# kuleshov-group/PlantCaduceus

Measured on AMD Instinct MI355X. Metric: 512-bp sequences/sec (zero-shot logits), PlantCaduceus_l32, higher is better.
Workload: dtype bf16; 1 GPU; PlantCaduceus_l32 (d_model=1024, n_layer=32) bf16 zero-shot SNP scoring: masked-LM forward of 1024 synthetic 512-bp windows per GPU per step (both strands), logits at index 255 -> softmax(a,c,g,t); synthetic checkpoint seed 1234; batch_per_gpu=1024, seq_len=512, parallelism=dp1 (batch-sharded, all_gather of [B,4])

## Files before the change

### plantcaduceus_amd/csrc/api.hip

```cpp
#include <cstdarg>
#include <cstdio>
#include <cstdlib>
#include <cstring>
#include <map>
#include <string>

#include "build_hash.h"
#include "pcad_internal.hpp"

using namespace pcad;

static thread_local char g_err[512] = "";

int pcad::fail(int code, const char* fmt, ...) {
    va_list ap;
    va_start(ap, fmt);
    vsnprintf(g_err, sizeof(g_err), fmt, ap);
    va_end(ap);
    return code;
}

int pcad::positions_arg(const char* who, const int32_t* positions, int P, int L, Positions* pos) {
    if (P < 0 || P > PCAD_MAX_POSITIONS || (P > 0 && !positions)) return fail(PCAD_ERR_INVALID, "%s: bad positions (P=%d)", who, P);
    pos->n = P;
    for (int i = 0; i < 16; ++i) pos->p[i] = 0;
    for (int i = 0; i < P; ++i) {
        if (positions[i] < 0 || positions[i] >= L) return fail(PCAD_ERR_INVALID, "%s: position %d out of range [0,%d)", who, positions[i], L);
        pos->p[i] = positions[i];
    }
    return PCAD_OK;
}

int pcad::probs_cols_arg(const char* who, const int32_t* cols, int vocab, ProbCols* out) {
    if (!cols) return fail(PCAD_ERR_INVALID, "%s: null cols", who);
    for (int j = 0; j < 4; ++j) {
        if (cols[j] < 0 || cols[j] >= vocab) return fail(PCAD_ERR_INVALID, "%s: cols[%d]=%d outside [0, %d)", who, j, cols[j], vocab);
        out->c[j] = cols[j];
    }
    return PCAD_OK;
}

struct Carver {
    char* base;
    size_t off = 0;
    explicit Carver(void* b) : base((char*)b) {}
    void* take(size_t bytes) {
        void* p = base ? base + off : nullptr;
        off += align_up(bytes);
        return p;
    }
};

bool pcad::fold_wanted(const pcad_engine* e) {
    const bool want = e->norm_fold == 1 || (e->norm_fold < 0 && e->cfg.dtype == PCAD_BF16);
    return want && !e->untied && e->rdt == F32 && e->xzsplit && e->blocked;
}

bool pcad::split_wanted(const pcad_engine* e) {
    return e->f32_split && e->cfg.dtype == PCAD_F32 && !fold_wanted(e) && e->xzsplit && e->blocked && e->D % 64 == 0 && e->E % 64 == 0;
}

static int64_t chunk_row_limit(const pcad_engine* e) {
    const int64_t per_row = (int64_t)e->E * e->esz;
    return ((((int64_t)1 << 32) - ((int64_t)2 << 20)) / per_row) & ~(int64_t)7;
}

static void carve_weights(pcad_engine* e, Carver& c) {
    const size_t D = e->D, E = e->E, N = e->N, V = e->V, esz = e->esz;
    const bool pf = fold_wanted(e);
    const bool ps = split_wanted(e);
    e->emb = c.take(V * D * esz);
    e->emb_f32 = (float*)c.take(V * D * 4);
    e->normf_w = (float*)c.take(D * 4);
    e->comp = (int32_t*)c.take(8 * 4);
    e->xz_tab0 = pf ? c.take(V * 2 * E * esz) : nullptr;
    e->layers.resize(e->nl);
    for (auto& L : e->layers) {
        L.norm_w = (float*)c.take(D * 4);
        L.convw = (float*)c.take(convx_packed_bytes((int)E, e->cfg.dtype));
        L.W_in = c.take(2 * E * D * esz);
        L.W_in_f = pf ? c.take(2 * E * D * esz) : nullptr;
        L.W_out = c.take(D * E * esz);
        L.W_out_p = pf && (size_t)fold_padded_width((int)D) != D ? c.take((size_t)fold_padded_width((int)D) * E * esz) : L.W_out;
        L.W_in_s = ps ? c.take(2 * E * 2 * D * 2) : nullptr;
        L.W_out_s = ps ? c.take(D * 2 * E * 2) : nullptr;
        L.W_in_r = e->untied ? c.take(2 * E * D * esz) : nullptr;
        L.W_out_r = e->untied ? c.take(D * E * esz) : nullptr;
        L.W_in_s_r = e->untied && ps ? c.take(2 * E * 2 * D * 2) : nullptr;
        L.W_out_s_r = e->untied && ps ? c.take(D * 2 * E * 2) : nullptr;
        for (int d = 0; d < 2; ++d) {
            DirWeights& w = L.dir[d];
            w.conv_w = (float*)c.take(E * 4 * 4);
            w.conv_b = (float*)c.take(E * 4);
            w.Wx = c.take((size_t)e->XP * E * esz);
            w.Wx_s = ps && e->convx ? c.take((size_t)e->XP * 2 * E * 2) : nullptr;
            w.Wdt = c.take(E * (size_t)e->Rp * esz);
            w.Wdt_s = ps && e->convx ? c.take(E * (size_t)e->Rp * 2 * 2) : nullptr;
            w.dt_bias = (float*)c.take(E * 4);
            w.A2 = (float*)c.take(E * N * 4);
            w.Dskip = (float*)c.take(E * 4);
        }
    }
}

SmallForms pcad::small_forms(const pcad_engine* e, int B, int L) {
    SmallForms f;
    if (!e->segments) return f;
    f.G = scan_segments(2 * B, L, e->E, nullptr);
    f.pair = e->convx && scan_pair_wanted(2 * B, L, e->E);
    f.ksplit = e->convx ? convx_ksplit(2 * B, L, e->E, e->cfg.dtype) : 1;
    return f;
}

Workspace pcad::carve_workspace(const pcad_engine* e, void* base, int Bc, int L, int Bpol) {
    Carver c(base);
    const size_t rows = (size_t)2 * Bc * L;
    const size_t D = e->D, E = e->E, esz = e->esz;
    Workspace w;
    const size_t Dp = fold_padded_width((int)D);
    w.res = c.take(rows * Dp * (e->rdt == F32 ? 4 : esz));
    const bool sp = split_wanted(e);
    w.u = c.take(rows * Dp * esz);
    w.h = c.take(rows * D * esz);
    const size_t rows8 = (rows + 7) / 8 * 8;
    w.xz = c.take((e->xzsplit ? rows8 : rows * 2) * E * esz);
    w.zb = e->xzsplit ? c.take(rows8 * E * esz) : nullptr;
    w.xc[0] = c.take(rows8 * E * esz);
    w.xc[1] = c.take(rows8 * E * esz);
    const size_t dtl_bytes = sp && e->convx ? rows * e->Rp * 2 * 2 : rows * e->Rp * esz;
    w.dtl[0] = c.take(dtl_bytes);
    w.dtl[1] = c.take(dtl_bytes);
    w.bc[0] = (float*)c.take(rows * 2 * e->N * 4);
    w.bc[1] = (float*)c.take(rows * 2 * e->N * 4);
    w.y = c.take(rows8 * E * esz);
    w.ys = sp ? c.take(rows8 * 2 * E * 2) : nullptr;
    w.rstd = (float*)c.take(rows * 4);
    w.ssq = (float*)c.take(rows * (Dp / 128) * 4);
    const SmallForms f = small_forms(e, Bpol, L);
    w.seg = f.G > 1 ? (float*)c.take(scan_segment_bytes(2 * Bc, L, (int)E, 2 * Bpol)) : nullptr;
    w.pair = f.pair ? (float*)c.take(scan_pair_bytes(2 * Bc, (int)E)) : nullptr;
    w.cxp = f.ksplit > 1 ? (float*)c.take(convx_split_bytes(2 * Bc, L, (int)E, e->cfg.dtype, e->Rp, 2 * Bpol)) : nullptr;
    w.xz2 = e->untied ? c.take((e->xzsplit ? rows8 : rows * 2) * E * esz) : nullptr;
    w.zb2 = e->untied && e->xzsplit ? c.take(rows8 * E * esz) : nullptr;
    w.bytes = c.off;
    return w;
}

static const char* const kClassNames[PCAD_NUM_KERNEL_CLASSES] = {
    "add_rmsnorm", "gemm_in_proj", "conv1d_bidir", "gemm_x_proj", "selective_scan", "gemm_out_proj", "final_head",
    "gemm_out_proj_res", "rstd_reduce"};

hipEvent_t pcad::prof_event(pcad_engine* e) {
    if (!e->prof_pool.empty()) {
        hipEvent_t ev = e->prof_pool.back();
        e->prof_pool.pop_back();
        return ev;
    }
    hipEvent_t ev = nullptr;
    if (hipEventCreate(&ev) != hipSuccess) return nullptr;
    return ev;
}

static const pcad_tensor* find(const std::map<std::string, const pcad_tensor*>& m, const std::string& k) {
    auto it = m.find(k);
    return it == m.end() ? nullptr : it->second;
}

static int64_t numel(const pcad_tensor* t) {
    int64_t n = 1;
    for (int i = 0; i < t->ndim; ++i) n *= t->shape[i];
    return n;
}

int pcad::chunk_for(const pcad_engine* e, int B, int L) {
    int64_t cap = chunk_row_limit(e) / (2 * (int64_t)L);
    if (e->chunk > 0 && e->chunk < cap) cap = e->chunk;
    if (cap < 1) cap = 1;
    if (cap > B) cap = B;
    if (e->ws_limit > 0 && carve_workspace(e, nullptr, (int)cap, L, B).bytes > (size_t)e->ws_limit) {
        int64_t lo = 1, hi = cap;
        while (lo < hi) {
            const int64_t mid = (lo + hi + 1) / 2;
            if (carve_workspace(e, nullptr, (int)mid, L, B).bytes <= (size_t)e->ws_limit) lo = mid; else hi = mid - 1;
        }
        cap = lo;
    }
    int64_t n = (B + cap - 1) / cap;
    if (e->chunk == 0 && e->ws_limit == 0) {
        auto whole = [&](int64_t m) { const int64_t c = (B + m - 1) / m; return (2 * c * (int64_t)L) % 16384 == 0; };
        if (!whole(n))
            for (int64_t m = n + 1; m <= 2 * n && m <= B; ++m)
                if (whole(m)) { n = m; break; }
    }
    return (int)((B + n - 1) / n);
}

extern "C" {

int pcad_version(void) { return PCAD_VERSION; }
const char* pcad_build_hash(void) { return PCAD_BUILD_HASH; }
const char* pcad_last_error(void) { return g_err; }

int pcad_create(const pcad_config* cfg, pcad_handle* out) {
    if (!cfg || !out) return fail(PCAD_ERR_INVALID, "pcad_create: null argument");
    if (cfg->d_state != 16) return fail(PCAD_ERR_INVALID, "d_state=%d unsupported (16 only)", cfg->d_state);
    if (cfg->d_conv != 4) return fail(PCAD_ERR_INVALID, "d_conv=%d unsupported (4 only)", cfg->d_conv);
    if (cfg->vocab != 8) return fail(PCAD_ERR_INVALID, "padded vocab=%d unsupported (8 only)", cfg->vocab);
    if (cfg->d_model <= 0 || cfg->d_model % 64 || cfg->d_model > 2048)
        return fail(PCAD_ERR_INVALID, "d_model=%d must be a multiple of 64, <= 2048", cfg->d_model);
    if (cfg->expand < 1) return fail(PCAD_ERR_INVALID, "expand=%d must be >= 1", cfg->expand);
    if (cfg->n_layer < 1) return fail(PCAD_ERR_INVALID, "n_layer=%d must be >= 1", cfg->n_layer);
    if (cfg->dt_rank < 1 || cfg->dt_rank > 256) return fail(PCAD_ERR_INVALID, "dt_rank=%d must be in 1 .. 256", cfg->dt_rank);
    if (cfg->dtype != PCAD_F32 && cfg->dtype != PCAD_BF16) return fail(PCAD_ERR_INVALID, "bad dtype %d", cfg->dtype);
    for (int i = 0; i < 8; ++i)
        if (cfg->complement[i] < 0 || cfg->complement[i] > 7) return fail(PCAD_ERR_INVALID, "bad complement map");
    pcad_engine* e = new pcad_engine();
    e->cfg = *cfg;
    e->D = cfg->d_model; e->E = cfg->expand * cfg->d_model; e->N = 16; e->R = cfg->dt_rank; e->V = 8;
    e->nl = cfg->n_layer;
    e->Rp = padded_dt_rank(e->R);
    e->XP = e->Rp + 2 * e->N;
    e->esz = cfg->dtype == PCAD_BF16 ? 2 : 4;
    e->rdt = (cfg->residual_in_fp32 || cfg->dtype == PCAD_F32) ? F32 : BF16;
    const char* ck = dev_env("PCAD_CHUNK_SEQS");
    e->chunk = ck ? atoi(ck) : 0;
    if (e->chunk < 0) e->chunk = 0;
    e->chunk_rows = 0;
    e->blocked = dev_env("PCAD_PLAIN_LAYOUT") == nullptr && (e->E * e->esz) % 128 == 0;
    e->xzsplit = e->blocked && dev_env("PCAD_PLAIN_XZ") == nullptr && e->E % 16 == 0;
    e->convx = e->xzsplit && (e->Rp == 64 || e->Rp == 96) && dev_env("PCAD_NO_CONVX") == nullptr;
    e->gate_once = true;
    *out = e;
    return PCAD_OK;
}

void pcad_destroy(pcad_handle h) {
    if (!h) return;
    for (int c = 0; c < PCAD_NUM_KERNEL_CLASSES; ++c)
        for (auto& pr : h->prof_ev[c]) { (void)hipEventDestroy(pr.first); (void)hipEventDestroy(pr.second); }
    for (auto ev : h->prof_pool) (void)hipEventDestroy(ev);
    delete h;
}

int pcad_set_option(pcad_handle h, const char* key, int64_t value) {
    if (!h || !key) return fail(PCAD_ERR_INVALID, "pcad_set_option: null argument");
    const std::string k(key);
    if (k == "chunk_seqs") {
        if (value < 0 || value > (1 << 20)) return fail(PCAD_ERR_INVALID, "chunk_seqs=%lld out of range", (long long)value);
        h->chunk = (int)value;
    } else if (k == "gate_each") {
        h->gate_once = value == 0;
    } else if (k == "norm_fold") {
        h->norm_fold = value < 0 ? -1 : (value != 0 ? 1 : 0);
    } else if (k == "workspace_limit_mb") {
        if (value < 0 || value > ((int64_t)1 << 30)) return fail(PCAD_ERR_INVALID, "workspace_limit_mb=%lld out of range", (long long)value);
        h->ws_limit = value << 20;
    } else if (k == "f32_gemm_split") {
        h->f32_split = value != 0;
    } else if (k == "untied_directions") {
        h->untied = value != 0;
    } else if (k == "reference_order") {
        if (value < 0 || value > 2) return fail(PCAD_ERR_INVALID, "reference_order=%lld out of range (0, 1, 2)", (long long)value);
        h->ref_order = (int)value;
        h->gate_once = value == 0;
        h->norm_fold = value == 0 ? -1 : 0;
    } else if (k == "debug_repeat_class") {
        if (value < -1 || value >= PCAD_NUM_KERNEL_CLASSES) return fail(PCAD_ERR_INVALID, "debug_repeat_class=%lld out of range", (long long)value);
        h->rep_class = (int)value;
    } else if (k == "debug_repeat") {
        if (value < 1 || value > 10000) return fail(PCAD_ERR_INVALID, "debug_repeat=%lld out of range", (long long)value);
        h->rep_count = (int)value;
    } else if (k == "poison_workspace") {
        h->poison = value != 0;
    } else if (k == "scan_segments") {
        h->segments = value != 0;
    } else if (k == "last_layer_shortcut") {
        h->shortcut = value != 0;
    } else {
        return fail(PCAD_ERR_INVALID, "pcad_set_option: unknown option '%s'", key);
    }
    return PCAD_OK;
}

int pcad_set_status_buffer(pcad_handle h, int32_t* status) {
    if (!h) return fail(PCAD_ERR_INVALID, "pcad_set_status_buffer: null handle");
    if (((uintptr_t)status) % 4) return fail(PCAD_ERR_INVALID, "pcad_set_status_buffer: misaligned pointer");
    h->status = status;
    return PCAD_OK;
}

size_t pcad_weight_arena_bytes(pcad_handle h) {
    if (!h) return 0;
    pcad_engine tmp = *h;
    Carver c(nullptr);
    carve_weights(&tmp, c);
    return c.off;
}

int pcad_bind_weights(pcad_handle h, const pcad_tensor* tensors, int n, void* arena, size_t arena_bytes,
                      pcad_stream stream) {
    if (!h || !tensors || !arena) return fail(PCAD_ERR_INVALID, "pcad_bind_weights: null argument");
    if (((uintptr_t)arena) % 256) return fail(PCAD_ERR_WORKSPACE, "weight arena must be 256-byte aligned");
    if (arena_bytes < pcad_weight_arena_bytes(h))
        return fail(PCAD_ERR_WORKSPACE, "weight arena too small: %zu < %zu", arena_bytes, pcad_weight_arena_bytes(h));
    hipStream_t s = (hipStream_t)stream;
    pcad_engine* e = h;
    Carver c(arena);
    carve_weights(e, c);
    std::map<std::string, const pcad_tensor*> m;
    for (int i = 0; i < n; ++i) {
        if (!tensors[i].name || !tensors[i].data) return fail(PCAD_ERR_INVALID, "tensor %d has null name/data", i);
        if (tensors[i].dtype != PCAD_F32 && tensors[i].dtype != PCAD_BF16)
            return fail(PCAD_ERR_INVALID, "tensor %s: bad dtype", tensors[i].name);
        m[tensors[i].name] = &tensors[i];
    }
    const int D = e->D, E = e->E, N = e->N, R = e->R, Rp = e->Rp, V = e->V, dt = e->cfg.dtype;
    const std::string pre = "caduceus.backbone.";

    auto need = [&](const std::string& k, int64_t expect, const char* missing_fmt = nullptr) -> const pcad_tensor* {
        const pcad_tensor* t = find(m, k);
        if (!t) {
            if (missing_fmt) fail(PCAD_ERR_INVALID, missing_fmt, k.c_str()); else fail(PCAD_ERR_MISSING, "missing tensor %s", k.c_str());
            return nullptr;
        }
        if (numel(t) != expect) {
            fail(PCAD_ERR_INVALID, "tensor %s has %lld elements, expected %lld", k.c_str(), (long long)numel(t),
                 (long long)expect);
            return nullptr;
        }
        return t;
    };
#define NEED(var, key, ...)                              \
    const pcad_tensor* var = need((key), __VA_ARGS__);   \
    if (!var) return g_err[0] == 'm' ? PCAD_ERR_MISSING : PCAD_ERR_INVALID

    NEED(t_emb, pre + "embeddings.word_embeddings.embedding.weight", (int64_t)V * D);
    HIP_TRY(launch_pack2d(t_emb->data, t_emb->dtype, D, e->emb, dt, D, V, D, V, D, s));
    HIP_TRY(launch_pack2d(e->emb, dt, D, e->emb_f32, F32, D, V, D, V, D, s));
    NEED(t_nf, pre + "norm_f.weight", (int64_t)D);
    HIP_TRY(launch_pack2d(t_nf->data, t_nf->dtype, D, e->normf_w, F32, D, 1, D, 1, D, s));
    HIP_TRY(hipMemcpyAsync(e->comp, e->cfg.complement, 8 * sizeof(int32_t), hipMemcpyHostToDevice, s));

    for (int i = 0; i < e->nl; ++i) {
        LayerWeights& L = e->layers[i];
        const std::string lp = pre + "layers." + std::to_string(i) + ".";
        NEED(t_norm, lp + "norm.weight", (int64_t)D);
        HIP_TRY(launch_pack2d(t_norm->data, t_norm->dtype, D, L.norm_w, F32, D, 1, D, 1, D, s));
        const std::string mf = lp + "mixer.submodule.mamba_fwd.";
        NEED(t_in, mf + "in_proj.weight", (int64_t)2 * E * D);
        HIP_TRY(launch_pack2d(t_in->data, t_in->dtype, D, L.W_in, dt, D, 2 * E, D, 2 * E, D, s));
        if (L.W_in_f) HIP_TRY(launch_pack_scale_cols(t_in->data, t_in->dtype, D, L.norm_w, L.W_in_f, dt, D, 2 * E, D, s));
        NEED(t_out, mf + "out_proj.weight", (int64_t)D * E);
        HIP_TRY(launch_pack2d(t_out->data, t_out->dtype, E, L.W_out, dt, E, D, E, D, E, s));
        if (L.W_out_p != L.W_out) HIP_TRY(launch_pack2d(t_out->data, t_out->dtype, E, L.W_out_p, dt, E, D, E, fold_padded_width(D), E, s));
        if (L.W_in_s) HIP_TRY(launch_pack_split_w(t_in->data, t_in->dtype, D, L.W_in_s, 2 * E, D, s));
        if (L.W_out_s) HIP_TRY(launch_pack_split_w(t_out->data, t_out->dtype, E, L.W_out_s, D, E, s));
        if (e->untied) {
            const std::string mr = lp + "mixer.submodule.mamba_rev.";
            NEED(t_in_r, mr + "in_proj.weight", (int64_t)2 * E * D, "\"untied_directions\" 1 needs tensor %s");
            NEED(t_out_r, mr + "out_proj.weight", (int64_t)D * E, "\"untied_directions\" 1 needs tensor %s");
            HIP_TRY(launch_pack2d(t_in_r->data, t_in_r->dtype, D, L.W_in_r, dt, D, 2 * E, D, 2 * E, D, s));
            HIP_TRY(launch_pack2d(t_out_r->data, t_out_r->dtype, E, L.W_out_r, dt, E, D, E, D, E, s));
            if (L.W_in_s_r) HIP_TRY(launch_pack_split_w(t_in_r->data, t_in_r->dtype, D, L.W_in_s_r, 2 * E, D, s));
            if (L.W_out_s_r) HIP_TRY(launch_pack_split_w(t_out_r->data, t_out_r->dtype, E, L.W_out_s_r, D, E, s));
        }
        for (int d = 0; d < 2; ++d) {
            DirWeights& w = L.dir[d];
            const std::string mp = lp + "mixer.submodule.mamba_" + (d == 0 ? "fwd." : "rev.");
            NEED(t_cw, mp + "conv1d.weight", (int64_t)E * 4);
            HIP_TRY(launch_pack2d(t_cw->data, t_cw->dtype, 4, w.conv_w, F32, 4, E, 4, E, 4, s));
            NEED(t_cb, mp + "conv1d.bias", (int64_t)E);
            HIP_TRY(launch_pack2d(t_cb->data, t_cb->dtype, E, w.conv_b, F32, E, 1, E, 1, E, s));
            NEED(t_x, mp + "x_proj.weight", (int64_t)(R + 2 * N) * E);
            const size_t esz_src = t_x->dtype == PCAD_BF16 ? 2 : 4;
            HIP_TRY(launch_pack2d(t_x->data, t_x->dtype, E, w.Wx, dt, E, R, E, Rp, E, s));
            HIP_TRY(launch_pack2d((const char*)t_x->data + (size_t)R * E * esz_src, t_x->dtype, E,
                                  (char*)w.Wx + (size_t)Rp * E * e->esz, dt, E, 2 * N, E, 2 * N, E, s));
            if (w.Wx_s) HIP_TRY(launch_pack_convx_wsplit((const float*)w.Wx, E, w.Wx_s, e->XP, E, s));
            NEED(t_dw, mp + "dt_proj.weight", (int64_t)E * R);
            HIP_TRY(launch_pack2d(t_dw->data, t_dw->dtype, R, w.Wdt, dt, Rp, E, R, E, Rp, s));
            if (w.Wdt_s) HIP_TRY(launch_pack_split_w(w.Wdt, dt, Rp, w.Wdt_s, E, Rp, s));
            NEED(t_db, mp + "dt_proj.bias", (int64_t)E);
            HIP_TRY(launch_pack2d(t_db->data, t_db->dtype, E, w.dt_bias, F32, E, 1, E, 1, E, s));
            NEED(t_A, mp + "A_log", (int64_t)E * N);
            HIP_TRY(launch_pack_A(t_A->data, t_A->dtype, w.A2, (int64_t)E * N, 1.4426950408889634f, s));
            NEED(t_D, mp + "D", (int64_t)E);
            HIP_TRY(launch_pack2d(t_D->data, t_D->dtype, E, w.Dskip, F32, E, 1, E, 1, E, s));
        }
        if ((E * e->esz) % 128 == 0)
            HIP_TRY(launch_pack_convw(L.dir[0].conv_w, L.dir[0].conv_b, L.dir[1].conv_w, L.dir[1].conv_b, L.convw, E, dt, s));
    }
#undef NEED
    if (e->xz_tab0) HIP_TRY(launch_embed_inproj_table(e->emb, e->layers[0].W_in_f, e->xz_tab0, V, D, 2 * E, e->cfg.eps, dt, s));
    e->fold_packed = fold_wanted(e);
    e->split_packed = split_wanted(e);
    e->untied_packed = e->untied;
    e->bound = true;
    return PCAD_OK;
}

size_t pcad_workspace_bytes(pcad_handle h, int batch, int seqlen) {
    if (!h || batch <= 0 || seqlen <= 0) return 0;
    return carve_workspace(h, nullptr, chunk_for(h, batch, seqlen), seqlen, batch).bytes;
}

int pcad_profile_enable(pcad_handle h, int on) {
    if (!h) return fail(PCAD_ERR_INVALID, "pcad_profile_enable: null handle");
    h->prof = on != 0;
    h->prof_stride = on > 1 ? on : 1;
    for (int c = 0; c < PCAD_NUM_KERNEL_CLASSES; ++c) h->prof_seen[c] = 0;
    return PCAD_OK;
}

int pcad_profile_read(pcad_handle h, pcad_kernel_stat* out, int max_out) {
    if (!h || !out) return fail(PCAD_ERR_INVALID, "pcad_profile_read: null argument");
    for (int c = 0; c < PCAD_NUM_KERNEL_CLASSES; ++c) {
        for (auto& pr : h->prof_ev[c]) {
            HIP_TRY(hipEventSynchronize(pr.second));
            float ms = 0.f;
            HIP_TRY(hipEventElapsedTime(&ms, pr.first, pr.second));
            h->prof_ms[c] += ms;
            h->prof_n[c] += 1;
            h->prof_pool.push_back(pr.first);
            h->prof_pool.push_back(pr.second);
        }
        h->prof_ev[c].clear();
    }
    int n = 0;
    for (int c = 0; c < PCAD_NUM_KERNEL_CLASSES && n < max_out; ++c, ++n) {
        snprintf(out[n].name, sizeof(out[n].name), "%s", kClassNames[c]);
        out[n].launches = h->prof_n[c];
        out[n].total_ms = h->prof_ms[c];
        h->prof_n[c] = 0;
        h->prof_ms[c] = 0.0;
    }
    return n;
}
}
```

### plantcaduceus_amd/csrc/forward.hip

```cpp
#include "pcad_internal.hpp"
using namespace pcad;

namespace {
enum class Head { lm, pooled, loss, probs, layers };
struct ForwardRequest {
    Head head = Head::lm;
    const int32_t* ids = nullptr; int B = 0, L = 0;
    void* workspace = nullptr; size_t ws_bytes = 0; pcad_stream stream = nullptr;
    const int32_t* positions = nullptr; int P = 0;
    const int32_t* pos_per_window = nullptr; int Pw = 0;
    void* all_hidden = nullptr;
    void* hidden_out = nullptr; float* logits_out = nullptr;
    struct {
        int pooling, num_labels;
        const float* score_w; float *pooled_out, *logits_out;
    } pool = {};
    struct {
        const int32_t* labels; const float* loss_weights; int ignore_index;
        float *sums_out, *nll_out, *logits_out;
    } loss = {};
    struct {
        ProbCols cols; float *probs_out, *logits_out;
    } probs = {};
    struct {
        const int32_t* layers;
        int NL;
        bool inter, average;
        int top;
        void* out;
    } lay = {};
};

struct ForwardPlan {
    int chunk, nchunks;
    bool fold, sp, untied;
    bool lay_inter, strict;
    int depth;
    int walk_len;
    SmallForms forms;
    bool tab0;
    int Q;
};

ForwardPlan plan_forward(const pcad_engine* e, const ForwardRequest& rq, const Positions& pos) {
    const int B = rq.B, L = rq.L, D = e->D, E = e->E, P = rq.P;
    ForwardPlan pl;
    pl.Q = rq.pos_per_window ? rq.Pw : (P ? P : L);
    pl.chunk = chunk_for(e, B, L);
    pl.nchunks = (B + pl.chunk - 1) / pl.chunk;
    pl.lay_inter = rq.head == Head::layers && rq.lay.inter;
    pl.fold = fold_wanted(e) && e->fold_packed && !rq.all_hidden && !pl.lay_inter;
    for (int ck = 0; ck < pl.nchunks && pl.fold; ++ck) {
        const int Bc = (B - ck * pl.chunk) < pl.chunk ? (B - ck * pl.chunk) : pl.chunk;
        pl.fold = gemm_fold_shapes_ok((int64_t)2 * Bc * L, D, E, e->cfg.dtype);
    }
    pl.untied = e->untied && e->untied_packed;
    pl.sp = split_wanted(e) && e->split_packed;
    pl.strict = (e->ref_order == 2 || pl.untied) && !pl.fold;
    pl.forms = small_forms(e, B, L);
    pl.depth = pl.lay_inter && rq.lay.top < e->nl ? rq.lay.top : e->nl;
    const bool truncated = pl.depth < e->nl;
    pl.walk_len = 0;
    if (e->shortcut && P > 0 && !rq.pos_per_window && !rq.all_hidden && (int64_t)P * E <= (int64_t)L * D &&
        (truncated ? pl.depth > 0 && !(pl.forms.pair && !pl.strict) : !pl.lay_inter)) {
        int pmin = pos.p[0], pmax = pos.p[0];
        for (int i = 1; i < P; ++i) { pmin = pos.p[i] < pmin ? pos.p[i] : pmin; pmax = pos.p[i] > pmax ? pos.p[i] : pmax; }
        const int need = (pmax + 1 > L - pmin) ? pmax + 1 : L - pmin;
        pl.walk_len = (need + 7) / 8 * 8;
        if (pl.walk_len > L) pl.walk_len = L;
    }
    static const bool tab0 = dev_env("PCAD_NO_TAB0") == nullptr;
    pl.tab0 = tab0;
    return pl;
}

struct Lane { Workspace w; int b0, Bc; };
struct Walk {
    pcad_engine* const e;
    const ForwardRequest& rq; const ForwardPlan& pl; const Positions& pos; const hipStream_t s;
    const int B, L, P, D, E, N, Rp, XP, dt, rdt;
    const int Dp;
    const size_t esz; const float eps;
    const int layP;
    Walk(pcad_engine* e_, const ForwardRequest& rq_, const ForwardPlan& pl_, const Positions& pos_)
        : e(e_), rq(rq_), pl(pl_), pos(pos_), s((hipStream_t)rq_.stream), B(rq_.B), L(rq_.L), P(rq_.P), D(e_->D), E(e_->E), N(e_->N),
          Rp(e_->Rp), XP(e_->XP), dt(e_->cfg.dtype), rdt(e_->rdt), Dp(fold_padded_width(e_->D)), esz(e_->esz), eps(e_->cfg.eps),
          layP(rq_.head == Head::layers ? pl_.Q : 0) {}
    int reps(int cls) const { return e->rep_class == cls ? e->rep_count : 1; }
    bool convx_fused(int64_t rows) const { return !pl.untied && e->convx && (rows + 16) * E * (int64_t)esz < ((int64_t)1 << 32); }
    bool dts(int64_t rows) const { return pl.sp && convx_fused(rows); }
    bool last_short(int li) const { return pl.walk_len > 0 && li + 1 == pl.depth; }
    bool truncated() const { return pl.depth < e->nl; }
    bool ys_from_scan(int li) const { return pl.sp && !pl.strict && !last_short(li) && L % 8 == 0 && e->blocked && e->xzsplit && pl.forms.G == 1; }
    bool pair(int64_t rows, int li) const { return pl.forms.pair && !pl.strict && li + 1 < e->nl && !last_short(li) && convx_fused(rows) && reps(PCAD_K_SCAN) == 1; }
    void* y_rev(const Lane& c) const { return pl.strict ? c.w.xc[0] : c.w.y; }
    const int32_t* ids_of(const Lane& c) const { return rq.ids + (int64_t)c.b0 * L; }
    const int32_t* ppw_of(const Lane& c) const { return rq.pos_per_window ? rq.pos_per_window + (size_t)c.b0 * rq.Pw : nullptr; }
    HeadInput head_in(const Lane& c) const {
        return {.h = c.w.h, .res = c.w.res, .w = e->normf_w, .B = c.Bc, .L = L, .D = D, .eps = eps, .dt = dt, .rdt = rdt, .res_frag = pl.fold ? Dp : 0,
                .ids = ids_of(c), .status = e->status};
    }
    hipError_t gather_rows(const Lane& c, const void* src) const {
        return launch_gather_rows({.src = src, .out = c.w.u, .B = c.Bc, .L = L, .E = E, .pos = pos, .dt = dt, .blocked = e->blocked}, s);
    }
    hipError_t out_proj(const Lane& c, int li, const void* src, int64_t n_rows, void* dst, int d, bool a_blocked) const {
        const LayerWeights& W = e->layers[li];
        const void *Wo = pl.untied && d ? W.W_out_r : W.W_out, *Wo_s = pl.untied && d ? W.W_out_s_r : W.W_out_s;
        if (pl.sp) {
            if (!(ys_from_scan(li) && src == c.w.y))
                if (hipError_t er = launch_split_rows((const float*)src, E, c.w.ys, n_rows, E, a_blocked, a_blocked, s)) return er;
            return launch_gemm_nt({.A = c.w.ys, .lda = 2 * E, .W = Wo_s, .ldw = 2 * E, .M = n_rows, .N = D, .K = 3 * E, .dt = BF16, .a_blocked = a_blocked, .ksplit = E / 64},
                                  {.C = dst, .ldc = D, .out_dt = F32}, s);
        }
        return launch_gemm_nt({.A = src, .lda = E, .W = Wo, .ldw = E, .M = n_rows, .N = D, .K = E, .dt = dt, .a_blocked = a_blocked}, {.C = dst, .ldc = D, .out_dt = dt}, s);
    }
    hipError_t in_proj(const Lane& c, const LayerWeights& W, int64_t rows, int d, void* x, void* z) const {
        if (pl.sp)
            return launch_gemm_nt_two({.A = c.w.u, .lda = 2 * D, .W = d ? W.W_in_s_r : W.W_in_s, .ldw = 2 * D, .M = rows, .N = 2 * E, .K = 3 * D, .dt = BF16, .ksplit = D / 64},
                                      {.C1 = x, .C2 = z, .nsplit = E, .out_blocked = true, .out_dt = F32}, s);
        const GemmOperands g{.A = c.w.u, .lda = D, .W = d ? W.W_in_r : W.W_in, .ldw = D, .M = rows, .N = 2 * E, .K = D, .dt = dt};
        if (e->xzsplit) return launch_gemm_nt_two(g, {.C1 = x, .C2 = z, .nsplit = E, .out_blocked = true}, s);
        return launch_gemm_nt(g, {.C = x, .ldc = 2 * E, .out_dt = dt}, s);
    }
    int64_t ldxz() const { return e->xzsplit ? E : 2 * E; }
    ScanDirection scan_dir(const Lane& c, const LayerWeights& W, int d, bool dts) const {
        const DirWeights& dw = W.dir[d];
        return {.u = c.w.xc[d], .dt_low = c.w.dtl[d], .Wdt = dts ? dw.Wdt_s : dw.Wdt, .bc = c.w.bc[d], .A2 = dw.A2, .Dskip = dw.Dskip, .dbias = dw.dt_bias};
    }
    int64_t lddt(bool dts) const { return dts ? 2 * Rp : Rp; }
    ScanLaunch scan_of(const Lane& c, const LayerWeights& W, int d, bool dts) const {
        return {.dir = scan_dir(c, W, d, dts), .ldz = ldxz(), .lddt = lddt(dts), .Rp = Rp, .y = c.w.y, .S = 2 * c.Bc, .L = L, .E = E, .dt = dt,
                .uy_blocked = e->blocked, .z_blocked = e->xzsplit, .seg_ws = c.w.seg, .dt_split = dts,
                .policy_S = 2 * B};
    }
    int lay_slot(int level) const {
        if (rq.head != Head::layers) return -1;
        if (!rq.lay.layers) return level;
        for (int i = 0; i < rq.lay.NL; ++i)
            if (rq.lay.layers[i] == level) return i;
        return -1;
    }
    void* lay_dst(int slot, int b0) const {
        return (char*)rq.lay.out + ((size_t)slot * B + b0) * layP * (rq.lay.average ? (size_t)D * 4 : (size_t)2 * D * esz);
    }
    int emit_level(Lane& c, int level, bool compact = false) const {
        if (rq.all_hidden) {
            char* dst = (char*)rq.all_hidden + ((size_t)level * B * L * 2 * D + (size_t)c.b0 * L * 2 * D) * esz;
            HIP_TRY(launch_assemble_hidden(c.w.h, dst, c.Bc, L, D, dt, s));
        }
        const int slot = lay_slot(level);
        if (slot >= 0)
            HIP_TRY(launch_layer_rows({.src = c.w.h, .out = lay_dst(slot, c.b0), .B = c.Bc, .L = L, .D = D, .dt = dt, .pos = pos, .pos_per_window = ppw_of(c), .P = layP,
                                       .average = rq.lay.average, .compact = compact, .status = e->status}, s));
        return PCAD_OK;
    }
    int fits_dead(const Lane& c, size_t need, const char* who, const char* what, size_t shown = 0) const {
        const size_t avail = (size_t)((char*)rq.workspace + c.w.bytes - (char*)c.w.xz);
        if (need > avail) return fail(PCAD_ERR_WORKSPACE, "%s: the %s (%zu bytes) do not fit the dead buffers (%zu)", who, what, shown ? shown : need, avail);
        return PCAD_OK;
    }
    int level0(Lane& c) const {
        if (pl.fold || !(rq.all_hidden || lay_slot(0) >= 0)) return PCAD_OK;
        HIP_TRY(launch_embed_only(ids_of(c), e->emb, e->comp, c.w.h, c.Bc, L, D, dt, s));
        return emit_level(c, 0);
    }
    int add_norm(Lane& c, int li) const {
        const LayerWeights& W = e->layers[li];
        const EmbedRows emb{.ids = ids_of(c), .emb = e->emb, .comp8 = e->comp, .B = c.Bc, .L = L};
        if (pl.fold) {
            if (li == 0) {
                ProfScope ps(e, PCAD_K_NORM, s);
                HIP_TRY(launch_embed_rmsnorm({.w = W.norm_w, .y = pl.tab0 ? nullptr : c.w.u, .res_out = c.w.res, .D = D, .eps = eps, .dt = dt, .rdt = rdt, .rstd_out = c.w.rstd, .Dp = Dp}, emb, s));
            }
            return PCAD_OK;
        }
        if (li == 0) {
            ProfScope ps(e, PCAD_K_NORM, s);
            HIP_TRY(launch_embed_rmsnorm({.w = W.norm_w, .y = c.w.u, .res_out = c.w.res, .D = D, .eps = eps, .dt = dt, .rdt = rdt, .split_y = pl.sp}, emb, s));
        } else {
            ProfScope ps(e, PCAD_K_NORM, s);
            HIP_TRY(launch_add_rmsnorm({.x = c.w.h, .res_in = c.w.res, .w = W.norm_w, .y = c.w.u, .res_out = c.w.res, .rows = (int64_t)2 * c.Bc * L, .D = D, .eps = eps, .dt = dt, .rdt = rdt,
                                        .split_y = pl.sp}, s));
        }
        return PCAD_OK;
    }
    int in_proj_conv(Lane& c, int li) const {
        const LayerWeights& W = e->layers[li];
        const int S = 2 * c.Bc;
        const int64_t rows = (int64_t)S * L;
        const bool sp = pl.sp;
        if (pl.untied) {
            for (int d = 0; d < 2; ++d) {
                void *xd = d ? c.w.xz2 : c.w.xz, *zd = d ? c.w.zb2 : c.w.zb;
                { ProfScope ps(e, PCAD_K_GEMM_IN, s);
                HIP_TRY(in_proj(c, W, rows, d, xd, zd)); }
                ProfScope ps(e, PCAD_K_CONV, s);
                ConvLaunch cv{.x = xd, .ldx = ldxz(), .ldy = E, .S = S, .L = L, .E = E, .dt = dt, .in_blocked = e->xzsplit, .out_blocked = e->blocked};
                const bool reverse = d == 1;
                ConvDirection& side = reverse ? cv.rev : cv.fwd;
                side = {.w = W.dir[d].conv_w, .b = W.dir[d].conv_b, .y = c.w.xc[d]};
                HIP_TRY(launch_conv_dir(cv, reverse, s));
            }
            return PCAD_OK;
        }
        if (pl.fold && li == 0 && pl.tab0) {
            ProfScope ps(e, PCAD_K_NORM, s);
            HIP_TRY(launch_embed_xz_gather(ids_of(c), e->comp, e->xz_tab0, c.w.xz, c.w.zb, c.Bc, L, E, dt, s));
        } else
        for (int rep = 0; rep < reps(PCAD_K_GEMM_IN); ++rep)
        { ProfScope ps(e, PCAD_K_GEMM_IN, s);
        if (pl.fold)
            HIP_TRY(launch_gemm_nt_two({.A = c.w.u, .lda = Dp, .W = W.W_in_f, .ldw = D, .M = rows, .N = 2 * E, .K = D, .dt = dt},
                                       {.C1 = c.w.xz, .C2 = c.w.zb, .nsplit = E, .out_blocked = true, .rscale = c.w.rstd}, s));
        else HIP_TRY(in_proj(c, W, rows, 0, c.w.xz, c.w.zb)); }
        if (convx_fused(rows)) for (int rep = 0; rep < reps(PCAD_K_CONV); ++rep) {
            ProfScope ps(e, PCAD_K_CONV, s);
            ConvxLaunch cx{.x = c.w.xz, .convw = W.convw, .S = S, .L = L, .E = E, .dt = dt, .Rp = Rp,
                           .dtl_split = sp,
                           .w_split = sp, .part_ws = c.w.cxp, .policy_S = 2 * B};
            for (int d = 0; d < 2; ++d) cx.dir[d] = {.Wx = sp ? W.dir[d].Wx_s : W.dir[d].Wx, .xc = c.w.xc[d], .dtl = c.w.dtl[d], .bc = c.w.bc[d]};
            HIP_TRY(launch_convx(cx, s));
        } else {
            ProfScope ps(e, PCAD_K_CONV, s);
            HIP_TRY(launch_conv_bidir({.x = c.w.xz, .ldx = ldxz(), .fwd = {.w = W.dir[0].conv_w, .b = W.dir[0].conv_b, .y = c.w.xc[0]},
                                       .rev = {.w = W.dir[1].conv_w, .b = W.dir[1].conv_b, .y = c.w.xc[1]}, .S = S, .L = L, .E = E, .dt = dt,
                                       .in_blocked = e->xzsplit, .out_blocked = e->blocked}, s));
        }
        return PCAD_OK;
    }
    int scans(Lane& c, int li) const {
        const LayerWeights& W = e->layers[li];
        const int S = 2 * c.Bc;
        const int64_t rows = (int64_t)S * L;
        const bool dts = this->dts(rows), strict = pl.strict, ys_from_scan = this->ys_from_scan(li);
        if (pair(rows, li)) {
            ScanPairLaunch pw{.fwd = scan_dir(c, W, 0, dts), .rev = scan_dir(c, W, 1, dts), .z = c.w.zb, .lddt = lddt(dts), .Rp = Rp, .y = c.w.y,
                              .S = S, .L = L, .E = E, .dt = dt, .gate_each = !e->gate_once, .ws = c.w.pair, .ysplit = ys_from_scan ? c.w.ys : nullptr,
                              .dt_split = dts};
            for (int ph = 1; ph <= 2; ++ph) {
                ProfScope ps(e, PCAD_K_SCAN, s);
                pw.phases = ph;
                HIP_TRY(launch_scan_pair(pw, s));
            }
            return PCAD_OK;
        }
        for (int d = 0; d < 2; ++d) {
            const DirWeights& dw = W.dir[d];
            if (!convx_fused(rows)) { ProfScope ps(e, PCAD_K_GEMM_X, s);
            HIP_TRY(launch_gemm_nt_split({.A = c.w.xc[d], .lda = E, .W = dw.Wx, .ldw = E, .M = rows, .N = XP, .K = E, .dt = dt, .a_blocked = e->blocked},
                                         {.C = c.w.dtl[d], .ldc = Rp, .C2 = c.w.bc[d], .ldc2 = 2 * N, .nsplit = Rp}, s)); }
            const ScanLaunch base = scan_of(c, W, d, dts);
            for (int rep = 1; rep < (d == 0 ? reps(PCAD_K_SCAN) : 1); ++rep)
                HIP_TRY(launch_scan(base, s));
            ProfScope ps(e, PCAD_K_SCAN, s);
            const void* zp = e->xzsplit ? c.w.zb : (const void*)((const char*)c.w.xz + (size_t)E * esz);
            if (pl.untied && d == 1) zp = e->xzsplit ? c.w.zb2 : (const void*)((const char*)c.w.xz2 + (size_t)E * esz);
            const bool gated = strict || !e->gate_once || d == 1;
            ScanLaunch sc = base;
            sc.z = gated ? zp : nullptr;
            sc.y = d == 1 ? y_rev(c) : c.w.y;
            sc.reverse = d == 1;
            sc.accumulate = strict ? 0 : (d == 1 ? (e->gate_once ? 2 : 1) : 0);
            sc.walk_len = last_short(li) ? pl.walk_len : 0;
            sc.ysplit = d == 1 && ys_from_scan ? c.w.ys : nullptr;
            HIP_TRY(launch_scan(sc, s));
        }
        return PCAD_OK;
    }
    int out_proj_strict(Lane& c, int li) const {
        const int S = 2 * c.Bc;
        const int64_t rows = (int64_t)S * L;
        if (last_short(li)) {
            ProfScope ps(e, PCAD_K_HEAD, s);
            HIP_TRY(gather_rows(c, c.w.y));
            HIP_TRY(out_proj(c, li, c.w.u, (int64_t)S * P, c.w.h, 0, false));
            HIP_TRY(gather_rows(c, y_rev(c)));
            HIP_TRY(out_proj(c, li, c.w.u, (int64_t)S * P, c.w.xz, 1, false));
            HIP_TRY(launch_add_round(c.w.h, c.w.xz, (int64_t)S * P * D, dt, s));
            return truncated() ? emit_level(c, li + 1, true) : PCAD_OK;
        }
        { ProfScope ps(e, PCAD_K_GEMM_OUT, s);
        HIP_TRY(out_proj(c, li, c.w.y, rows, c.w.h, 0, e->blocked)); }
        { ProfScope ps(e, PCAD_K_GEMM_OUT, s);
        HIP_TRY(out_proj(c, li, y_rev(c), rows, c.w.u, 1, e->blocked)); }
        { ProfScope ps(e, PCAD_K_NORM, s);
        HIP_TRY(launch_add_round(c.w.h, c.w.u, rows * D, dt, s)); }
        return li + 1 < e->nl ? emit_level(c, li + 1) : PCAD_OK;
    }
    int out_proj_shortcut(Lane& c, int li) const {
        ProfScope ps(e, PCAD_K_HEAD, s);
        HIP_TRY(gather_rows(c, c.w.y));
        HIP_TRY(out_proj(c, li, c.w.u, (int64_t)2 * c.Bc * P, c.w.h, 0, false));
        return truncated() ? emit_level(c, li + 1, true) : PCAD_OK;
    }
    int out_proj_folded(Lane& c, int li) const {
        const LayerWeights& W = e->layers[li];
        const int64_t rows = (int64_t)2 * c.Bc * L;
        { ProfScope ps(e, PCAD_K_GEMM_OUT_RES, s);
        HIP_TRY(launch_gemm_nt_res({.A = c.w.y, .lda = E, .W = W.W_out_p, .ldw = E, .M = rows, .N = Dp, .K = E, .dt = dt, .a_blocked = e->blocked},
                                   {.C = c.w.u, .res = (float*)c.w.res, .ssq = c.w.ssq}, s)); }
        ProfScope ps(e, PCAD_K_RSTD, s);
        HIP_TRY(launch_rstd(c.w.ssq, c.w.rstd, rows, Dp / 128, D, eps, s));
        return PCAD_OK;
    }
    int out_proj_plain(Lane& c, int li) const {
        for (int rep = 0; rep < reps(PCAD_K_GEMM_OUT); ++rep)
        { ProfScope ps(e, PCAD_K_GEMM_OUT, s);
        HIP_TRY(out_proj(c, li, c.w.y, (int64_t)2 * c.Bc * L, c.w.h, 0, e->blocked)); }
        return li + 1 < e->nl ? emit_level(c, li + 1) : PCAD_OK;
    }
    int mixer_out(Lane& c, int li) const {
        return pl.strict ? out_proj_strict(c, li) : last_short(li) ? out_proj_shortcut(c, li)
               : pl.fold && li + 1 < e->nl ? out_proj_folded(c, li) : out_proj_plain(c, li);
    }
    int head_lm(Lane& c) const {
        void* hout = rq.hidden_out ? (char*)rq.hidden_out + ((size_t)c.b0 * pl.Q * 2 * D) * esz : nullptr;
        float* lout = rq.logits_out ? rq.logits_out + (size_t)c.b0 * pl.Q * e->V : nullptr;
        if (!hout && !lout) return PCAD_OK;
        ProfScope ps(e, PCAD_K_HEAD, s);
        HIP_TRY(launch_final_head({.in = head_in(c), .emb_f32 = e->emb_f32, .comp8 = e->comp, .hidden_out = hout, .logits_out = lout, .pos = pos,
                                   .pos_per_seq = ppw_of(c), .h_compact = pl.walk_len > 0}, s));
        return PCAD_OK;
    }
    int head_pooled(Lane& c) const {
        const auto& pool = rq.pool;
        const size_t part = pool_partial_bytes(c.Bc, L, D, pool.pooling);
        if (int rc = fits_dead(c, part, "pcad_forward_pooled", "head's partials")) return rc;
        ProfScope ps(e, PCAD_K_HEAD, s);
        HIP_TRY(launch_pooled_head({.in = head_in(c), .score_w = pool.score_w, .NL = pool.num_labels, .pooled_out = pool.pooled_out ? pool.pooled_out + (size_t)c.b0 * 2 * D : nullptr,
                                    .logits_out = pool.logits_out + (size_t)c.b0 * pool.num_labels, .pooling = pool.pooling, .part = c.w.xz}, s));
        return PCAD_OK;
    }
    int head_loss(Lane& c) const {
        const auto& loss = rq.loss;
        if (int rc = fits_dead(c, loss_partial_bytes(c.Bc, L), "pcad_forward_loss", "head's partials")) return rc;
        const size_t o = (size_t)c.b0 * L;
        ProfScope ps(e, PCAD_K_HEAD, s);
        HIP_TRY(launch_loss_head({.in = head_in(c), .emb_f32 = e->emb_f32, .comp8 = e->comp, .labels = loss.labels + o, .loss_w = loss.loss_weights ? loss.loss_weights + o : nullptr,
                                  .ignore_index = loss.ignore_index, .sums_out = loss.sums_out + (size_t)c.b0 * 4, .nll_out = loss.nll_out ? loss.nll_out + o : nullptr,
                                  .logits_out = loss.logits_out ? loss.logits_out + o * e->V : nullptr, .part = c.w.xz}, s));
        return PCAD_OK;
    }
    int head_probs(Lane& c) const {
        const auto& probs = rq.probs; const int Qp = pl.Q;
        ProfScope ps(e, PCAD_K_HEAD, s);
        HIP_TRY(launch_probs_head({.in = head_in(c), .emb_f32 = e->emb_f32, .comp8 = e->comp, .cols = probs.cols,
                                   .probs_out = probs.probs_out ? probs.probs_out + (size_t)c.b0 * Qp * 4 : nullptr,
                                   .logits_out = probs.logits_out ? probs.logits_out + (size_t)c.b0 * Qp * e->V : nullptr, .pos = pos, .pos_per_window = ppw_of(c),
                                   .Pw = rq.Pw, .h_compact = pl.walk_len > 0}, s));
        return PCAD_OK;
    }
    int head_layers(Lane& c) const {
        const int32_t* ppw = ppw_of(c);
        char* rows_tmp = (char*)c.w.xz;
        const size_t slot_bytes = (size_t)c.Bc * 2 * D * esz, rows_bytes = align_up(slot_bytes * layP);
        const bool columns = ppw && layP > 1;
        if (int rc = fits_dead(c, rows_bytes + (columns ? align_up((size_t)c.Bc * layP * 4) : 0), "pcad_forward_layers", "last level's rows", rows_bytes)) return rc;
        const int slot = lay_slot(e->nl);
        auto emit = [&](int64_t sb, int64_t sq) {
            return launch_layer_rows({.src = rows_tmp, .out = lay_dst(slot, c.b0), .B = c.Bc, .L = L, .D = D, .dt = dt, .pos = pos, .P = layP, .assembled = true, .sb = sb, .sq = sq,
                                      .average = rq.lay.average}, s);
        };
        FinalHeadLaunch fh{.in = head_in(c), .emb_f32 = e->emb_f32, .comp8 = e->comp, .hidden_out = rows_tmp, .pos = pos, .h_compact = pl.walk_len > 0};
        ProfScope ps(e, PCAD_K_HEAD, s);
        if (ppw) {
            const int32_t* col = ppw;
            if (columns) {
                col = (const int32_t*)(rows_tmp + rows_bytes);
                HIP_TRY(launch_position_columns(ppw, (int32_t*)(rows_tmp + rows_bytes), c.Bc, layP, s));
            }
            fh.h_compact = false;
            for (int q = 0; q < layP; ++q) {
                fh.hidden_out = rows_tmp + slot_bytes * q;
                fh.pos_per_seq = col + (size_t)q * c.Bc;
                HIP_TRY(launch_final_head(fh, s));
            }
            if (slot >= 0) HIP_TRY(emit(1, c.Bc));
        } else {
            HIP_TRY(launch_final_head(fh, s));
            if (slot >= 0) HIP_TRY(emit(layP, 1));
        }
        return PCAD_OK;
    }
    int ids_check(Lane& c) const {
        ProfScope ps(e, PCAD_K_HEAD, s);
        HIP_TRY(launch_ids_check(ids_of(c), (int64_t)c.Bc * L, e->status, s));
        return PCAD_OK;
    }
    int head(Lane& c) const {
        if (truncated()) return ids_check(c);
        return rq.head == Head::pooled ? head_pooled(c) : rq.head == Head::loss ? head_loss(c) : rq.head == Head::probs ? head_probs(c)
               : rq.head == Head::layers ? head_layers(c) : head_lm(c);
    }
    int run() const {
        for (int ck = 0; ck < pl.nchunks; ++ck) {
            Lane c;
            c.b0 = ck * pl.chunk;
            c.Bc = (B - c.b0) < pl.chunk ? (B - c.b0) : pl.chunk;
            c.w = carve_workspace(e, rq.workspace, c.Bc, L, B);
            if (int rc = level0(c)) return rc;
            for (int li = 0; li < pl.depth; ++li) {
                if (int rc = add_norm(c, li)) return rc;
                if (int rc = in_proj_conv(c, li)) return rc;
                if (int rc = scans(c, li)) return rc;
                if (int rc = mixer_out(c, li)) return rc;
            }
            if (int rc = head(c)) return rc;
        }
        return PCAD_OK;
    }
};

int forward_impl(pcad_handle h, const ForwardRequest& rq) {
    if (!h) return fail(PCAD_ERR_INVALID, "pcad_forward: null handle");
    pcad_engine* e = h; const int B = rq.B, L = rq.L;
    if (!e->bound) return fail(PCAD_ERR_UNBOUND, "pcad_forward: weights not bound");
    if (B < 0 || L <= 0) return fail(PCAD_ERR_INVALID, "pcad_forward: bad B=%d L=%d", B, L);
    if (B == 0) return PCAD_OK;
    if (!rq.ids || !rq.workspace) return fail(PCAD_ERR_INVALID, "pcad_forward: null ids/workspace");
    Positions pos;
    if (int rc = positions_arg("pcad_forward", rq.positions, rq.P, L, &pos)) return rc;
    if (((uintptr_t)rq.workspace) % 256) return fail(PCAD_ERR_WORKSPACE, "workspace must be 256-byte aligned");
    const size_t need = pcad_workspace_bytes(h, B, L);
    if (rq.ws_bytes < need) return fail(PCAD_ERR_WORKSPACE, "workspace too small: %zu < %zu", rq.ws_bytes, need);
    if (e->poison) HIP_TRY(hipMemsetAsync(rq.workspace, 0xFF, need, (hipStream_t)rq.stream));
    if (fold_wanted(e) && !e->fold_packed)
        return fail(PCAD_ERR_INVALID, "pcad_forward: the norm-folded layer form (\"norm_fold\" %s) was enabled after pcad_bind_weights, under options that "
                                      "did not ask for it; its weight copies are packed at bind time - set \"norm_fold\" / \"reference_order\" before "
                                      "pcad_weight_arena_bytes / pcad_bind_weights (turning the form OFF afterwards is always possible)",
                    e->norm_fold == 1 ? "1" : "default");
    if (split_wanted(e) && !e->split_packed)
        return fail(PCAD_ERR_INVALID, "pcad_forward: \"f32_gemm_split\" 1 was set after pcad_bind_weights; the split weight copies are packed at "
                                      "bind time - set the option before pcad_weight_arena_bytes / pcad_bind_weights");
    if (e->untied && !e->untied_packed)
        return fail(PCAD_ERR_INVALID, "pcad_forward: \"untied_directions\" 1 was set after pcad_bind_weights; mamba_rev's in_proj / out_proj are packed at "
                                      "bind time - set the option before pcad_weight_arena_bytes / pcad_bind_weights");
    const ForwardPlan pl = plan_forward(e, rq, pos);
    return Walk(e, rq, pl, pos).run();
}

}

extern "C" {

int pcad_forward(pcad_handle h, const int32_t* ids, int B, int L, const int32_t* positions, int P, void* hidden_out,
                 float* logits_out, void* workspace, size_t workspace_bytes, pcad_stream stream) {
    ForwardRequest rq;
    rq.head = Head::lm; rq.ids = ids; rq.B = B; rq.L = L; rq.workspace = workspace; rq.ws_bytes = workspace_bytes; rq.stream = stream;
    rq.positions = positions; rq.P = P; rq.hidden_out = hidden_out; rq.logits_out = logits_out;
    return forward_impl(h, rq);
}

int pcad_forward_pooled(pcad_handle h, const int32_t* ids, int B, int L, int pooling, const float* score_w, int num_labels,
                        float* pooled_out, float* logits_out, void* workspace, size_t workspace_bytes, pcad_stream stream) {
    if (pooling < PCAD_POOL_MEAN || pooling > PCAD_POOL_LAST) return fail(PCAD_ERR_INVALID, "pcad_forward_pooled: bad pooling %d", pooling);
    if (num_labels < 1 || num_labels > PCAD_MAX_LABELS)
        return fail(PCAD_ERR_INVALID, "pcad_forward_pooled: num_labels=%d out of range [1, %d]", num_labels, PCAD_MAX_LABELS);
    if (!score_w || !logits_out) return fail(PCAD_ERR_INVALID, "pcad_forward_pooled: null score_w / logits_out");
    ForwardRequest rq;
    rq.head = Head::pooled; rq.ids = ids; rq.B = B; rq.L = L; rq.workspace = workspace; rq.ws_bytes = workspace_bytes; rq.stream = stream;
    rq.pool.pooling = pooling; rq.pool.score_w = score_w; rq.pool.num_labels = num_labels;
    rq.pool.pooled_out = pooled_out; rq.pool.logits_out = logits_out;
    return forward_impl(h, rq);
}

int pcad_forward_loss(pcad_handle h, const int32_t* ids, const int32_t* labels, const float* loss_weights, int ignore_index, int B,
                      int L, float* sums_out, float* nll_out, float* logits_out, void* workspace, size_t workspace_bytes,
                      pcad_stream stream) {
    if (!h) return fail(PCAD_ERR_INVALID, "pcad_forward_loss: null handle");
    if (B < 0 || L <= 0) return fail(PCAD_ERR_INVALID, "pcad_forward_loss: bad B=%d L=%d", B, L);
    if (B > 0 && (!labels || !sums_out)) return fail(PCAD_ERR_INVALID, "pcad_forward_loss: null labels / sums_out");
    ForwardRequest rq;
    rq.head = Head::loss; rq.ids = ids; rq.B = B; rq.L = L; rq.workspace = workspace; rq.ws_bytes = workspace_bytes; rq.stream = stream;
    rq.loss.labels = labels; rq.loss.loss_weights = loss_weights; rq.loss.ignore_index = ignore_index;
    rq.loss.sums_out = sums_out; rq.loss.nll_out = nll_out; rq.loss.logits_out = logits_out;
    return forward_impl(h, rq);
}

int pcad_forward_probs(pcad_handle h, const int32_t* ids, int B, int L, const int32_t* positions, int P, const int32_t* pos_per_window,
                       const int32_t* cols, float* probs_out, float* logits_out, void* workspace, size_t workspace_bytes,
                       pcad_stream stream) {
    if (!h) return fail(PCAD_ERR_INVALID, "pcad_forward_probs: null handle");
    if (positions && pos_per_window) return fail(PCAD_ERR_INVALID, "pcad_forward_probs: positions and pos_per_window are exclusive");
    if (P < 0 || P > PCAD_MAX_POSITIONS || (P > 0 && !positions && !pos_per_window) || (P == 0 && (positions || pos_per_window)))
        return fail(PCAD_ERR_INVALID, "pcad_forward_probs: bad positions (P=%d)", P);
    if (!probs_out && !logits_out) return fail(PCAD_ERR_INVALID, "pcad_forward_probs: no output requested");
    if (((uintptr_t)probs_out) % 16) return fail(PCAD_ERR_INVALID, "pcad_forward_probs: probs_out must be 16-byte aligned");
    ForwardRequest rq;
    rq.head = Head::probs; rq.ids = ids; rq.B = B; rq.L = L; rq.workspace = workspace; rq.ws_bytes = workspace_bytes; rq.stream = stream;
    if (int rc = probs_cols_arg("pcad_forward_probs", cols, h->V < PCAD_MAX_VOCAB ? h->V : PCAD_MAX_VOCAB, &rq.probs.cols)) return rc;
    rq.probs.probs_out = probs_out; rq.probs.logits_out = logits_out;
    if (pos_per_window) { rq.pos_per_window = pos_per_window; rq.Pw = P; } else { rq.positions = positions; rq.P = P; }
    return forward_impl(h, rq);
}

int pcad_forward_layers(pcad_handle h, const int32_t* ids, int B, int L, const int32_t* positions, int P, const int32_t* pos_per_window,
                        const int32_t* layers, int NL, int average, void* out, void* workspace, size_t workspace_bytes, pcad_stream stream) {
    if (!h) return fail(PCAD_ERR_INVALID, "pcad_forward_layers: null handle");
    if ((positions != nullptr) == (pos_per_window != nullptr))
        return fail(PCAD_ERR_INVALID, "pcad_forward_layers: exactly one of positions and pos_per_window (the all-positions form is pcad_forward_all_hidden)");
    if (P < 1 || P > PCAD_MAX_POSITIONS) return fail(PCAD_ERR_INVALID, "pcad_forward_layers: bad positions (P=%d)", P);
    const int nl = h->nl;
    if (layers ? (NL < 1 || NL > nl + 1) : NL != 0) return fail(PCAD_ERR_INVALID, "pcad_forward_layers: bad layers (NL=%d, n_layer=%d)", NL, nl);
    for (int i = 0; i < NL; ++i) {
        if (layers[i] < 0 || layers[i] > nl) return fail(PCAD_ERR_INVALID, "pcad_forward_layers: level %d outside [0, %d]", layers[i], nl);
        if (i > 0 && layers[i] <= layers[i - 1]) return fail(PCAD_ERR_INVALID, "pcad_forward_layers: levels must be strictly increasing");
    }
    if (!out || ((uintptr_t)out) % 16) return fail(PCAD_ERR_INVALID, "pcad_forward_layers: out must be a 16-byte aligned pointer");
    ForwardRequest rq;
    rq.head = Head::layers; rq.ids = ids; rq.B = B; rq.L = L; rq.workspace = workspace; rq.ws_bytes = workspace_bytes; rq.stream = stream;
    rq.lay.layers = layers; rq.lay.NL = layers ? NL : nl + 1; rq.lay.inter = !layers || layers[0] < nl;
    rq.lay.top = layers ? layers[NL - 1] : nl;
    rq.lay.average = average != 0; rq.lay.out = out;
    if (pos_per_window) { rq.pos_per_window = pos_per_window; rq.Pw = P; } else { rq.positions = positions; rq.P = P; }
    return forward_impl(h, rq);
}

int pcad_forward_at(pcad_handle h, const int32_t* ids, int B, int L, const int32_t* pos_per_seq, void* hidden_out,
                    float* logits_out, void* workspace, size_t workspace_bytes, pcad_stream stream) {
    if (!pos_per_seq) return fail(PCAD_ERR_INVALID, "pcad_forward_at: null pos_per_seq");
    ForwardRequest rq;
    rq.head = Head::lm; rq.ids = ids; rq.B = B; rq.L = L; rq.workspace = workspace; rq.ws_bytes = workspace_bytes; rq.stream = stream;
    rq.pos_per_window = pos_per_seq; rq.Pw = 1; rq.hidden_out = hidden_out; rq.logits_out = logits_out;
    return forward_impl(h, rq);
}

int pcad_forward_all_hidden(pcad_handle h, const int32_t* ids, int B, int L, void* all_hidden, void* hidden_out,
                            float* logits_out, void* workspace, size_t workspace_bytes, pcad_stream stream) {
    if (!all_hidden) return fail(PCAD_ERR_INVALID, "pcad_forward_all_hidden: null all_hidden");
    ForwardRequest rq;
    rq.head = Head::lm; rq.ids = ids; rq.B = B; rq.L = L; rq.workspace = workspace; rq.ws_bytes = workspace_bytes; rq.stream = stream;
    rq.all_hidden = all_hidden; rq.hidden_out = hidden_out; rq.logits_out = logits_out;
    return forward_impl(h, rq);
}

}
```

### plantcaduceus_amd/csrc/gemm.hip

```cpp
#include <cstdlib>
#include <type_traits>

#include "common.hpp"
#include "kernels.hpp"

namespace pcad {

typedef __bf16 bf16x8_t __attribute__((ext_vector_type(8)));

constexpr int BM = 256, BN = 128, ROWB = 128;
constexpr int A_BYTES = BM * ROWB, W_BYTES = BN * ROWB;
constexpr int STAGE_BYTES = A_BYTES + W_BYTES;
constexpr int NSTAGE = 3;
constexpr int GEMM_LDS = NSTAGE * STAGE_BYTES;
constexpr int GEMM_THREADS = 512;
#ifndef PCAD_WALK_CONST
#define PCAD_WALK_CONST 8
#endif
constexpr int walk = PCAD_WALK_CONST;

__device__ __forceinline__ int ksplit_a(int kt, int nk) { return kt >= 2 * nk ? kt - 2 * nk : kt; }
__device__ __forceinline__ int ksplit_w(int kt, int nk) { return kt >= nk ? kt - nk : kt; }
__device__ __forceinline__ int key_a(int r) { return (r >> 1) & 7; }
__device__ __forceinline__ int key_w(int r) { return (((r >> 4) & 3) << 1) | ((r >> 1) & 1); }
// ... 678 lines not shown
        constexpr int MODE = (int)decltype(first_tag)::value;
        constexpr bool FIRST = MODE == 1;
        constexpr int SLOT = (int)decltype(slot_tag)::value;
        const int abn = nsa * A2_BYTES, wbn = nsw * W2_BYTES, kx = nkk << 6;
        auto lda = [&](int f) __attribute__((always_inline)) { an[f] = *reinterpret_cast<const u32x4*>(smem + ((abn + a_fo[f]) ^ kx)); };
        auto ldw = [&](int f) __attribute__((always_inline)) { wn[f] = *reinterpret_cast<const u32x4*>(smem + ((wbn + w_fo[f]) ^ kx)); };
        auto dma = [&](int p) __attribute__((always_inline)) { if (dma_a) a_piece(dma_stage, p); else w_piece(dma_stage, p); };
#pragma unroll
        for (int r = 0; r < 8; ++r) {
            if constexpr (MODE == 2) {
                switch (r) {
                    case 0: wait_vmcnt_row<res_row_wait(0)>(acc[0]); break; case 1: wait_vmcnt_row<res_row_wait(1)>(acc[1]); break;
                    case 2: wait_vmcnt_row<res_row_wait(2)>(acc[2]); break; case 3: wait_vmcnt_row<res_row_wait(3)>(acc[3]); break;
                    case 4: wait_vmcnt_row<res_row_wait(4)>(acc[4]); break; case 5: wait_vmcnt_row<res_row_wait(5)>(acc[5]); break;
                    case 6: wait_vmcnt_row<res_row_wait(6)>(acc[6]); break; default: wait_vmcnt_row<res_row_wait(7)>(acc[7]); break;
                }
            }
#pragma unroll
            for (int ks = 0; ks < 4; ++ks) {
#pragma unroll
                for (int j = 2 * ks; j < 2 * ks + 2; ++j) {
                    if (FIRST) MmaAcc<T>::run0(wc[j], ac[r], acc[r][j]);
                    else MmaAcc<T>::run(wc[j], ac[r], acc[r][j]);
                }
                const int k = ks == SLOT ? kDmaSlot : (ks == kDmaSlot ? SLOT : ks);
                if (k == kDmaSlot) dma(r);
                else if (r < 4) {
                    if (k == 0) ldw(2 * r);
                    else if (k == 2) ldw(2 * r + 1);
                } else if (r == 4) {
                    if (k == 0) lda(6); else if (k == 2) lda(7);
                } else if (r == 5) {
                    if (k == 0) lda(0); else if (k == 2) lda(1); else lda(2);
                } else if (r == 6) {
                    if (k == 0) lda(3); else if (k == 2) lda(4); else lda(5);
                }
                __builtin_amdgcn_sched_barrier(0);
            }
        }
    };
    const int swap_fix = (((lg & 1) * 16 + (lg >> 1) * 8) - lg * 16) * 2;
    float rs[8];
    auto load_rscale = [&](int64_t m0) __attribute__((always_inline)) {
        if constexpr (EPI == EPI_SCALE) {
            const float* sb = epi.rscale + (m0 + wm * 128);
            const uint32_t vo = (uint32_t)li * 4u;
            gload_v32<0>(rs[0], vo, sb);   gload_v32<64>(rs[1], vo, sb);  gload_v32<128>(rs[2], vo, sb); gload_v32<192>(rs[3], vo, sb);
            gload_v32<256>(rs[4], vo, sb); gload_v32<320>(rs[5], vo, sb); gload_v32<384>(rs[6], vo, sb); gload_v32<448>(rs[7], vo, sb);
        }
    };
    const uint32_t res_vo = (uint32_t)lane * 16u;
    auto res_tile_base = [&](int64_t m0, int n0) __attribute__((always_inline)) -> float* {
        return epi.res + ((((m0 >> 8) * (int64_t)(N >> 8) + (n0 >> 8)) * 4 + wave) << 14);
    };
    auto load_res_group = [&](const float* tb, int i, int jg) __attribute__((always_inline)) {
        const float* sb = tb + (i * 2 + jg) * 1024;
        gload_a128<0>(acc[i][jg * 4 + 0], res_vo, sb);    gload_a128<1024>(acc[i][jg * 4 + 1], res_vo, sb);
        gload_a128<2048>(acc[i][jg * 4 + 2], res_vo, sb); gload_a128<3072>(acc[i][jg * 4 + 3], res_vo, sb);
    };
    auto epilogue = [&](int64_t m0, int n0) __attribute__((always_inline)) {
        const int64_t mrow = m0 + wm * 128 + li;
        float ss[8];
        float* res_tb = nullptr;
        if constexpr (EPI == EPI_SCALE) {
            wait_vmcnt_regs<16>(rs);
        }
        if constexpr (EPI == EPI_RES) {
#pragma unroll
            for (int i = 0; i < 8; ++i) ss[i] = 0.f;
            res_tb = res_tile_base(m0, n0);
        }
#pragma unroll
        for (int jg = 0; jg < 2; ++jg) {
            const int nbase = n0 + wn * 128 + jg * 64;
            char* lane_dst;
            int64_t row_step;
            if (C2 != nullptr) {
                const bool second = nbase >= nsplit;
                const int width = second ? N - nsplit : nsplit;
                const int col = (second ? nbase - nsplit : nbase) + lg * 16;
                char* base = reinterpret_cast<char*>(second ? C2 : C);
                if (out_blocked) {
                    lane_dst = base + blocked_off(mrow, (int64_t)col * sizeof(OutT), ((int64_t)width * sizeof(OutT)) >> 7);
                    row_step = 2 * ((((int64_t)width * sizeof(OutT)) >> 7) << 10);
                } else {
                    lane_dst = base + (mrow * width + col) * (int64_t)sizeof(OutT);
                    row_step = 16 * (int64_t)width * sizeof(OutT);
                }
            } else {
                lane_dst = reinterpret_cast<char*>(C) + (mrow * ldc + nbase + lg * 16) * (int64_t)sizeof(OutT);
                row_step = 16 * ldc * (int64_t)sizeof(OutT);
            }
#pragma unroll
            for (int i = 0; i < 8; ++i) {
                f32x4 t0 = acc[i][jg * 4 + 0], t1 = acc[i][jg * 4 + 1], t2 = acc[i][jg * 4 + 2], t3 = acc[i][jg * 4 + 3];
                asm volatile("" : "+v"(t0), "+v"(t1), "+v"(t2), "+v"(t3));
                if constexpr (EPI == EPI_RES) {
                    float* rdst = res_tb + (i * 2 + jg) * 1024 + lane * 4;
                    __builtin_nontemporal_store(t0, reinterpret_cast<f32x4*>(rdst));       __builtin_nontemporal_store(t1, reinterpret_cast<f32x4*>(rdst + 256));
                    __builtin_nontemporal_store(t2, reinterpret_cast<f32x4*>(rdst + 512)); __builtin_nontemporal_store(t3, reinterpret_cast<f32x4*>(rdst + 768));
#pragma unroll
                    for (int rr = 0; rr < 4; ++rr)
                        ss[i] = __builtin_fmaf(t0[rr], t0[rr], __builtin_fmaf(t1[rr], t1[rr], __builtin_fmaf(t2[rr], t2[rr], __builtin_fmaf(t3[rr], t3[rr], ss[i]))));
                    asm volatile("" : "+v"(ss[i]));
                }
                if constexpr (EPI == EPI_SCALE) { t0 *= rs[i]; t1 *= rs[i]; t2 *= rs[i]; t3 *= rs[i]; }
                float lo[8], hi[8];
#pragma unroll
                for (int rr = 0; rr < 4; ++rr) {
                    lo[rr] = t0[rr]; lo[4 + rr] = t1[rr];
                    hi[rr] = t2[rr]; hi[4 + rr] = t3[rr];
                }
                OutT* dst = reinterpret_cast<OutT*>(lane_dst + i * row_step);
                if constexpr (sizeof(OutT) == 2) {
                    if (epi_swap) {
                        u32x4 L, H;
#pragma unroll
                        for (int d = 0; d < 4; ++d) {
                            const auto sw = __builtin_amdgcn_permlane32_swap(pack_bf16x2(lo[2 * d], lo[2 * d + 1]), pack_bf16x2(hi[2 * d], hi[2 * d + 1]), false, false);
                            L[d] = sw[0]; H[d] = sw[1];
                        }
                        char* db = reinterpret_cast<char*>(dst) + swap_fix;
                        *reinterpret_cast<u32x4*>(db) = L;
                        *reinterpret_cast<u32x4*>(db + 64) = H;
                        __builtin_amdgcn_sched_barrier(0);
                        continue;
                    }
                }
                store8<OutT>(dst, lo);
                store8<OutT>(dst + 8, hi);
                __builtin_amdgcn_sched_barrier(0);
            }
        }
        if constexpr (EPI == EPI_RES) {
            const int np = N >> 7;
#pragma unroll
            for (int i = 0; i < 8; ++i) {
                float v = ss[i];
                v += __shfl_xor(v, 16, 64);
                v += __shfl_xor(v, 32, 64);
                if (lg == 0) epi.ssq[(mrow + i * 16) * np + (n0 >> 7) + wn] = v;
            }
        }
    };

    int tile = blockIdx.x;
    int64_t m0; int n0;
    tile_coords(tile, m0, n0);
    set_pa(m0);
    set_pw(n0);
    load_rscale(m0);
    a_issue(0); a_advance();
    w_issue(0); w_advance();
    a_issue(1); a_advance();
    w_issue(1); w_advance();
    asm volatile("s_waitcnt vmcnt(16)" ::: "memory");
    __builtin_amdgcn_s_barrier();
    asm volatile("" ::: "memory");
    u32x4 fa0[8], fw0[8], fa1[8], fw1[8];
    load_frags(0, 0, 0, fa0, fw0);
    int sa = 0, sw = 0, kt = 0;
    auto mainloop = [&](auto slot) __attribute__((always_inline)) {
    while (true) {
        const int sa_n = sa == 2 ? 0 : sa + 1;
        const int sa_f = sa == 0 ? 2 : sa - 1;
        if constexpr (EPI == EPI_RES) {
            if (kt == 0) {
                const float* tb = res_tile_base(m0, n0);
#pragma unroll
                for (int i = 0; i < 8; ++i) { load_res_group(tb, i, 0); load_res_group(tb, i, 1); }
                kstep(fa0, fw0, fa1, fw1, sa, sw, 1, true, sa_f, std::integral_constant<int, 2>{}, slot);
            } else {
                kstep(fa0, fw0, fa1, fw1, sa, sw, 1, true, sa_f, std::integral_constant<int, 0>{}, slot);
            }
        } else {
            if (kt == 0) kstep(fa0, fw0, fa1, fw1, sa, sw, 1, true, sa_f, std::integral_constant<int, 1>{}, slot);
            else kstep(fa0, fw0, fa1, fw1, sa, sw, 1, true, sa_f, std::integral_constant<int, 0>{}, slot);
        }
        a_advance();
        asm volatile("s_waitcnt vmcnt(8) lgkmcnt(0)" ::: "memory");
        __builtin_amdgcn_s_barrier();
        asm volatile("" ::: "memory");
        kstep(fa1, fw1, fa0, fw0, sa_n, sw ^ 1, 0, false, sw, std::integral_constant<int, 0>{}, slot);
        w_advance();
        sa = sa_n;
        sw ^= 1;
        if (kt + 1 < nkt) {
            ++kt;
        } else {
            epilogue(m0, n0);
            tile += gstride;
            if (tile >= nblk) break;
            tile_coords(tile, m0, n0);
            load_rscale(m0);
            kt = 0;
        }
    }
    };
#ifdef PCAD_GEMM_STAGGER
    if (wave == 0) mainloop(std::integral_constant<int, 0>{});
    else if (wave == 1) mainloop(std::integral_constant<int, 1>{});
    else if (wave == 2) mainloop(std::integral_constant<int, 2>{});
    else mainloop(std::integral_constant<int, 3>{});
#else
    mainloop(std::integral_constant<int, kDmaSlot>{});
#endif
    asm volatile("s_waitcnt vmcnt(0)" ::: "memory");
}

static int persistent_grid(int nblk) {
    const int cap = device_cu_count() / 8 * 8;
    return nblk < cap ? nblk : cap;
}

template <typename T, typename OutT, bool ROUND>
static hipError_t launch_gemm_t(const GemmOperands& g, void* C, int64_t ldc, hipStream_t s) {
    const int tiles_m = (int)((g.M + BM - 1) / BM), tiles_n = (g.N + BN - 1) / BN;
    const bool vec = ((ldc * (int64_t)sizeof(OutT)) % 16 == 0) && (((uintptr_t)C) % 16 == 0);
    const auto kfn = vec ? gemm_nt_kernel<T, OutT, ROUND, true, false> : gemm_nt_kernel<T, OutT, ROUND, false, false>;
    if (hipError_t ae = ensure_dynamic_lds((const void*)kfn, GEMM_LDS)) return ae;
    hipLaunchKernelGGL(kfn, dim3((unsigned)persistent_grid(tiles_m * tiles_n)), dim3(GEMM_THREADS), GEMM_LDS, s, (const T*)g.A, g.lda, (const T*)g.W, g.ldw,
                       (OutT*)C, ldc, g.M, g.N, g.K, tiles_m, tiles_n, (float*)nullptr, (int64_t)0, 0, (int)g.a_blocked, g.ksplit);
    return hipGetLastError();
}

template <typename T>
static hipError_t launch_gemm_split_t(const GemmOperands& g, const GemmSplitOut& o, hipStream_t s) {
    const int tiles_m = (int)((g.M + BM - 1) / BM), tiles_n = (g.N + BN - 1) / BN;
    const auto kfn = gemm_nt_kernel<T, T, false, true, true>;
    if (hipError_t ae = ensure_dynamic_lds((const void*)kfn, GEMM_LDS)) return ae;
    hipLaunchKernelGGL(kfn, dim3((unsigned)persistent_grid(tiles_m * tiles_n)), dim3(GEMM_THREADS), GEMM_LDS, s, (const T*)g.A, g.lda, (const T*)g.W, g.ldw,
                       (T*)o.C, o.ldc, g.M, g.N, g.K, tiles_m, tiles_n, o.C2, o.ldc2, o.nsplit, (int)g.a_blocked, 0);
    return hipGetLastError();
}

hipError_t launch_gemm_nt_split(const GemmOperands& g, const GemmSplitOut& o, hipStream_t s) {
    if (g.M <= 0 || g.N <= 0) return hipSuccess;
    const int esz = g.dt == BF16 ? 2 : 4;
    if (g.K <= 0 || (g.K * esz) % ROWB || o.nsplit % 16 || (g.N - o.nsplit) % 16 || g.ksplit) return hipErrorInvalidValue;
    if ((g.lda * esz) % 16 || (g.ldw * esz) % 16 || ((uintptr_t)g.A) % 16 || ((uintptr_t)g.W) % 16) return hipErrorInvalidValue;
    if ((o.ldc * esz) % 16 || ((uintptr_t)o.C) % 16 || (o.ldc2 * 4) % 16 || ((uintptr_t)o.C2) % 16) return hipErrorInvalidValue;
    if (g.a_blocked && (g.lda * esz) % 128) return hipErrorInvalidValue;
    return g.dt == BF16 ? launch_gemm_split_t<bf16_t>(g, o, s) : launch_gemm_split_t<float>(g, o, s);
}

template <typename T>
static bool quad_ok(int64_t lda, int64_t ldw, int64_t M, int N, bool two, int nsplit) {
    const int64_t esz_ = (int64_t)sizeof(T);
    return M % BM2 == 0 && N % BN2 == 0 && (!two || nsplit % 64 == 0) && M * lda * esz_ < ((int64_t)1 << 32) - 65536 &&
           (int64_t)N * ldw * esz_ < ((int64_t)1 << 32) - 65536;
}

struct Gemm256Out {
    void* C;  int64_t ldc;
    void* C2 = nullptr;  int nsplit = 0;
    bool out_blocked = false;
    int epi_kind = EPI_NONE;
    GemmEpi epi = {nullptr, nullptr, nullptr};
};

template <typename T, typename OutT>
static auto gemm256q_for(int epi_kind) -> decltype(&gemm256q_kernel<T, OutT, EPI_NONE>) {
    if constexpr (std::is_same<T, OutT>::value) {
        if (epi_kind == EPI_SCALE) return gemm256q_kernel<T, OutT, EPI_SCALE>;
        if (epi_kind == EPI_RES) return gemm256q_kernel<T, OutT, EPI_RES>;
    }
    return epi_kind == EPI_NONE ? gemm256q_kernel<T, OutT, EPI_NONE> : nullptr;
}

template <typename T, typename OutT = T>
static hipError_t launch_gemm256_t(const GemmOperands& g, const Gemm256Out& o, hipStream_t s) {
    const int tiles_m = (int)((g.M + BM2 - 1) / BM2), tiles_n = (g.N + BN2 - 1) / BN2;
    const dim3 grid((unsigned)persistent_grid(tiles_m * tiles_n));
    static const bool quad = dev_env("PCAD_GEMM_NOQUAD") == nullptr;
    static const bool epi_swap = dev_env("PCAD_GEMM_EPI_PLAIN") == nullptr;
    const bool qok = quad_ok<T>(g.lda, g.ldw, g.M, g.N, o.C2 != nullptr, o.nsplit);
    if (o.epi_kind != EPI_NONE && !qok) return hipErrorInvalidValue;
    if (o.epi_kind != EPI_NONE || (quad && qok)) {
        const auto kq = gemm256q_for<T, OutT>(o.epi_kind);
        if (!kq) return hipErrorInvalidValue;
        if (hipError_t ae = ensure_dynamic_lds((const void*)kq, GEMM3_LDS)) return ae;
        hipLaunchKernelGGL(kq, grid, dim3(GEMMQ_THREADS), GEMM3_LDS, s, (const T*)g.A, g.lda, (const T*)g.W, g.ldw, (OutT*)o.C, o.ldc, g.M, g.N, g.K,
                           tiles_m, tiles_n, (int)g.a_blocked, (OutT*)o.C2, o.nsplit, (int)o.out_blocked, (int)epi_swap, o.epi, g.ksplit);
        return hipGetLastError();
    }
    const auto kr = gemm256r_kernel<T, OutT>;
    if (hipError_t ae = ensure_dynamic_lds((const void*)kr, GEMM3_LDS)) return ae;
    hipLaunchKernelGGL(kr, grid, dim3(GEMM_THREADS), GEMM3_LDS, s, (const T*)g.A, g.lda, (const T*)g.W, g.ldw, (OutT*)o.C, o.ldc, g.M, g.N, g.K, tiles_m,
                       tiles_n, (int)g.a_blocked, (OutT*)o.C2, o.nsplit, (int)o.out_blocked, g.ksplit);
    return hipGetLastError();
}

static hipError_t launch_gemm256(const GemmOperands& g, int out_dt, const Gemm256Out& o, hipStream_t s) {
    if (g.dt == BF16 && out_dt == F32) return launch_gemm256_t<bf16_t, float>(g, o, s);
    return g.dt == BF16 ? launch_gemm256_t<bf16_t>(g, o, s) : launch_gemm256_t<float>(g, o, s);
}

hipError_t launch_gemm_nt_two(const GemmOperands& g, const GemmTwoOut& o, hipStream_t s) {
    if (g.M <= 0 || g.N <= 0) return hipSuccess;
    const int dt = g.dt, N = g.N, K = g.K, nsplit = o.nsplit, ksplit = g.ksplit;
    const int esz = dt == BF16 ? 2 : 4;
    const int out_dt = o.out_dt < 0 ? dt : o.out_dt;
    const int osz = out_dt == BF16 ? 2 : 4;
    if (K <= 0 || (K * esz) % ROWB || nsplit % 16 || N % 16 || nsplit <= 0 || nsplit >= N || g.a_blocked) return hipErrorInvalidValue;
    if ((g.lda * esz) % 16 || (g.ldw * esz) % 16 || ((uintptr_t)g.A) % 16 || ((uintptr_t)g.W) % 16) return hipErrorInvalidValue;
    if (((uintptr_t)o.C1) % 16 || ((uintptr_t)o.C2) % 16) return hipErrorInvalidValue;
    if (o.out_blocked && ((nsplit * osz) % 128 || ((N - nsplit) * osz) % 128)) return hipErrorInvalidValue;
    if (out_dt != dt) {
        if (dt != BF16 || out_dt != F32 || o.rscale) return hipErrorInvalidValue;
        if (ksplit && (ksplit < 0 || K != 3 * ksplit * (ROWB / 2))) return hipErrorInvalidValue;
    } else if (ksplit) {
        return hipErrorInvalidValue;
    }
    return launch_gemm256(g, out_dt, {.C = o.C1, .ldc = nsplit, .C2 = o.C2, .nsplit = nsplit, .out_blocked = o.out_blocked,
                                      .epi_kind = o.rscale ? EPI_SCALE : EPI_NONE, .epi = {o.rscale, nullptr, nullptr}}, s);
}

bool gemm_fold_shapes_ok(int64_t M, int D, int E, int dt) {
    const int64_t esz = dt == BF16 ? 2 : 4;
    const int Dp = fold_padded_width(D);
    const bool in_ok = dt == BF16 ? quad_ok<bf16_t>(Dp, D, M, 2 * E, true, E) : quad_ok<float>(Dp, D, M, 2 * E, true, E);
    const bool out_ok = dt == BF16 ? quad_ok<bf16_t>(E, E, M, Dp, false, 0) : quad_ok<float>(E, E, M, Dp, false, 0);
    return in_ok && out_ok && (D * esz) % ROWB == 0 && (E * esz) % ROWB == 0 && M * (int64_t)Dp * 4 < ((int64_t)1 << 32);
}

hipError_t launch_gemm_nt_res(const GemmOperands& g, const GemmResOut& o, hipStream_t s) {
    if (g.M <= 0 || g.N <= 0) return hipSuccess;
    const int esz = g.dt == BF16 ? 2 : 4;
    if (g.K <= 0 || (g.K * esz) % ROWB || !o.res || !o.ssq || !o.C || g.ksplit) return hipErrorInvalidValue;
    if ((g.lda * esz) % 16 || (g.ldw * esz) % 16 || ((uintptr_t)g.A) % 16 || ((uintptr_t)g.W) % 16 || ((uintptr_t)o.res) % 16) return hipErrorInvalidValue;
    if (g.a_blocked && (g.lda * esz) % 128) return hipErrorInvalidValue;
    return launch_gemm256(g, g.dt, {.C = o.C, .ldc = g.N, .epi_kind = EPI_RES, .epi = {nullptr, o.res, o.ssq}}, s);
}

hipError_t launch_gemm_nt(const GemmOperands& g, const GemmPlainOut& o, hipStream_t s) {
    if (g.M <= 0 || g.N <= 0) return hipSuccess;
    const int dt = g.dt, out_dt = o.out_dt, ksplit = g.ksplit;
    const int esz = dt == BF16 ? 2 : 4;
    if (g.K <= 0 || (g.K * esz) % ROWB) return hipErrorInvalidValue;
    if (ksplit && (ksplit < 0 || dt != BF16 || out_dt != F32 || o.round_bf16 || g.K != 3 * ksplit * (ROWB / 2))) return hipErrorInvalidValue;
    if ((g.lda * esz) % 16 || (g.ldw * esz) % 16 || ((uintptr_t)g.A) % 16 || ((uintptr_t)g.W) % 16)
        return hipErrorInvalidValue;
    if (g.a_blocked && (g.lda * esz) % 128) return hipErrorInvalidValue;
    static const bool no256 = dev_env("PCAD_GEMM_NO256") != nullptr;
    const int osz = out_dt == BF16 ? 2 : 4;
    const bool big = !no256 && g.M >= 2048 && g.N >= 512 && g.N % 16 == 0 && (out_dt == dt || (dt == BF16 && out_dt == F32 && !o.round_bf16)) &&
                     (o.ldc * osz) % 16 == 0 && ((uintptr_t)o.C) % 16 == 0;
    if (big) return launch_gemm256(g, out_dt, {.C = o.C, .ldc = o.ldc}, s);
    if (dt == BF16 && out_dt == BF16) return launch_gemm_t<bf16_t, bf16_t, false>(g, o.C, o.ldc, s);
    if (dt == BF16 && out_dt == F32)
        return o.round_bf16 ? launch_gemm_t<bf16_t, float, true>(g, o.C, o.ldc, s) : launch_gemm_t<bf16_t, float, false>(g, o.C, o.ldc, s);
    if (dt == F32 && out_dt == F32) return launch_gemm_t<float, float, false>(g, o.C, o.ldc, s);
    return hipErrorInvalidValue;
}

}
```

### plantcaduceus_amd/csrc/kernels.hpp

```cpp
#pragma once
#include <hip/hip_runtime.h>
#include <stdint.h>
#include <stdlib.h>

namespace pcad {

enum DType { F32 = 0, BF16 = 1 };

inline const char* dev_env(const char* name) {
    static const bool dev = [] { const char* d = getenv("PCAD_DEV"); return d && d[0] == '1'; }();
    return dev ? getenv(name) : nullptr;
}

hipError_t ensure_dynamic_lds(const void* kernel, int bytes);
int device_cu_count();

struct Positions {
    int n;
    int p[16];
};

struct NormLaunch {
    const void* x = nullptr;
    const void* res_in = nullptr;
    const float* w;
    void* y;
    void* res_out;
    int64_t rows = 0;
    int D;  float eps;  int dt, rdt;
    bool split_y = false;
    float* rstd_out = nullptr;
    int Dp = 0;
};
hipError_t launch_add_rmsnorm(const NormLaunch& n, hipStream_t s);
struct EmbedRows { const int32_t* ids;  const void* emb;  const int32_t* comp8;  int B, L; };
hipError_t launch_embed_rmsnorm(const NormLaunch& n, const EmbedRows& e, hipStream_t s);
hipError_t launch_rstd(const float* ssq, float* rstd, int64_t rows, int np, int D, float eps, hipStream_t s);

struct HeadInput {
    const void* h;
    const void* res;
    const float* w;
    int B, L, D;  float eps;  int dt, rdt;
    int res_frag = 0;
    const int32_t* ids = nullptr;
    int32_t* status = nullptr;
};
inline hipError_t head_input_check(const HeadInput& in) {
    if (in.D % 8 || in.D > 2048) return hipErrorInvalidValue;
    if ((in.dt != BF16 && in.dt != F32) || (in.rdt != F32 && in.rdt != in.dt)) return hipErrorInvalidValue;
    if (in.res_frag && (in.rdt != F32 || in.res_frag % 256 || in.res_frag < in.D || ((int64_t)2 * in.B * in.L) % 256)) return hipErrorInvalidValue;
    return hipSuccess;
}
struct FinalHeadLaunch {
    HeadInput in;
    const float* emb_f32;  const int32_t* comp8;
    void* hidden_out = nullptr;
    float* logits_out = nullptr;
    Positions pos = {};
    const int32_t* pos_per_seq = nullptr;
    bool h_compact = false;
};
hipError_t launch_final_head(const FinalHeadLaunch& a, hipStream_t s);
enum { POOL_MEAN = 0, POOL_MAX = 1, POOL_FIRST = 2, POOL_LAST = 3 };
int pool_segments(int L, int pooling);
size_t pool_partial_bytes(int B, int L, int D, int pooling);
struct PooledHeadLaunch {
    HeadInput in;
    const float* score_w = nullptr;  int NL = 0;
    float* pooled_out = nullptr;
    float* logits_out = nullptr;
    int pooling;
    void* part;
};
hipError_t launch_pooled_head(const PooledHeadLaunch& a, hipStream_t s);
constexpr int LOSS_SEG = 64;
int loss_segments(int L);
size_t loss_partial_bytes(int B, int L);
struct LossHeadLaunch {
    HeadInput in;
    const float* emb_f32;  const int32_t* comp8;
    const int32_t* labels;
    const float* loss_w = nullptr;
    int ignore_index;
    float* sums_out;
    float* nll_out = nullptr;
    float* logits_out = nullptr;
    void* part;
};
hipError_t launch_loss_head(const LossHeadLaunch& a, hipStream_t s);
struct ProbCols { int c[4]; };
struct ProbsHeadLaunch {
    HeadInput in;
    const float* emb_f32;  const int32_t* comp8;
    ProbCols cols;
    float* probs_out = nullptr;
    float* logits_out = nullptr;
    Positions pos = {};
    const int32_t* pos_per_window = nullptr;  int Pw = 0;
    bool h_compact = false;
};
hipError_t launch_probs_head(const ProbsHeadLaunch& a, hipStream_t s);
struct LayerRowsLaunch {
    const void* src;
    void* out;
    int B, L, D, dt;
    Positions pos = {};
    const int32_t* pos_per_window = nullptr;
    int P;
    bool assembled = false;
    int64_t sb = 0;
    int64_t sq = 0;
    bool average = false;
    bool compact = false;
    int32_t* status = nullptr;
};
hipError_t launch_layer_rows(const LayerRowsLaunch& a, hipStream_t s);
hipError_t launch_ids_check(const int32_t* ids, int64_t n, int32_t* status, hipStream_t s);
hipError_t launch_position_columns(const int32_t* src, int32_t* dst, int B, int P, hipStream_t s);
hipError_t launch_assemble_hidden(const void* h, void* out, int B, int L, int D, int dt, hipStream_t s);
hipError_t launch_embed_only(const int32_t* ids, const void* emb, const int32_t* comp8, void* h, int B, int L,
                             int D, int dt, hipStream_t s);
hipError_t launch_add_round(void* a, const void* b, int64_t n, int dt, hipStream_t s);

struct GemmOperands {
    const void* A;  int64_t lda;
    const void* W;  int64_t ldw;
    int64_t M;  int N, K;
    int dt;
    bool a_blocked = false;
    int ksplit = 0;
};
struct GemmPlainOut {
    void* C;  int64_t ldc;
    int out_dt;
    bool round_bf16 = false;
};
struct GemmSplitOut { void* C;  int64_t ldc;  float* C2;  int64_t ldc2;  int nsplit; };
struct GemmTwoOut {
    void *C1, *C2;  int nsplit;
    bool out_blocked = false;
    const float* rscale = nullptr;
    int out_dt = -1;
};
struct GemmResOut { void* C;  float* res;  float* ssq; };
hipError_t launch_gemm_nt(const GemmOperands& g, const GemmPlainOut& o, hipStream_t s);
hipError_t launch_gemm_nt_split(const GemmOperands& g, const GemmSplitOut& o, hipStream_t s);
hipError_t launch_gemm_nt_two(const GemmOperands& g, const GemmTwoOut& o, hipStream_t s);
hipError_t launch_gemm_nt_res(const GemmOperands& g, const GemmResOut& o, hipStream_t s);
bool gemm_fold_shapes_ok(int64_t M, int D, int E, int dt);
inline int fold_padded_width(int D) { return (D + 255) / 256 * 256; }

struct ConvDirection { const float* w;  const float* b;  void* y; };
struct ConvLaunch {
    const void* x;  int64_t ldx;
    ConvDirection fwd, rev;
    int64_t ldy = 0;
    int S, L, E, dt;
    bool in_blocked = false;
    bool out_blocked = false;
};
hipError_t launch_conv_bidir(const ConvLaunch& c, hipStream_t s);
hipError_t launch_conv_dir(const ConvLaunch& c, bool reverse, hipStream_t s);

size_t convx_packed_bytes(int E, int dt);
hipError_t launch_pack_convw(const float* wf, const float* bf, const float* wr, const float* br, float* out, int E, int dt,
                             hipStream_t s);
struct ConvxDirection { const void* Wx;  void* xc;  void* dtl;  float* bc; };
struct ConvxLaunch {
    const void* x;  const float* convw;
    ConvxDirection dir[2];
    int S, L, E, dt;
    int Rp = 64;
    bool dtl_split = false;
    bool w_split = false;
    float* part_ws = nullptr;
    int policy_S = 0;
};
hipError_t launch_convx(const ConvxLaunch& c, hipStream_t s);
int convx_ksplit(int S, int L, int E, int dt);
size_t convx_split_bytes(int S, int L, int E, int dt, int Rp, int policy_S = 0);
hipError_t launch_pack_convx_wsplit(const float* src, int64_t ld, void* dst, int rows, int E, hipStream_t s);
inline int padded_dt_rank(int R) { return R <= 64 ? 64 : (R + 31) / 32 * 32; }

struct ScanDirection { const void *u, *dt_low, *Wdt; const float *bc, *A2, *Dskip, *dbias; };
struct ScanLaunch {
    ScanDirection dir;
    const void* delta = nullptr;
    const void* z = nullptr;  int64_t ldz = 0;
    int64_t lddt = 0;  int Rp = 0;
    float a_scale = 1.0f;
    void* y;
    int S, L, E, dt;
    bool reverse = false;
    int accumulate = 0;
    bool uy_blocked = false;
    bool z_blocked = false;
    float* seg_ws = nullptr;
    int walk_len = 0;
    void* ysplit = nullptr;
    bool dt_split = false;
    int policy_S = 0;
};
hipError_t launch_scan(const ScanLaunch& a, hipStream_t s);

inline int scan_segments(int S, int L, int E, int* seg_blocks) {
    const int64_t waves = (int64_t)S * (E / 64);
    const int nblk = (L + 31) / 32;
    const int min_blocks = L >= 2048 ? 16 : 1;
    int G = 1;
    if (L >= 256 && waves > 0 && waves <= (L >= 2048 ? 768 : 512)) {
        G = (int)((2304 + waves - 1) / waves);
        if (G > (L >= 2048 ? 8 : 16)) G = L >= 2048 ? 8 : 16;
        if (G > nblk / min_blocks) G = nblk / min_blocks;
        if (G < 3) G = 1;
    }
    const int sb = (nblk + G - 1) / G;
    G = (nblk + sb - 1) / sb;
    if (seg_blocks) *seg_blocks = sb;
    return G;
}
inline size_t scan_segment_bytes(int S, int L, int E, int policy_S = 0) {
    const int G = scan_segments(policy_S > 0 ? policy_S : S, L, E, nullptr);
    return G > 1 ? (size_t)S * G * E * 17 * sizeof(float) : 0;
}

inline bool scan_pair_wanted(int S, int L, int E) {
    const int64_t waves = (int64_t)S * (E / 64);
    static const int64_t max_waves = [] { const char* v = dev_env("PCAD_PAIR_MAX_WAVES"); return v ? (int64_t)atoll(v) : (int64_t)3584; }();
    return L % 64 == 0 && L >= 128 && waves > 0 && waves <= max_waves && scan_segments(S, L, E, nullptr) == 1;
}
inline size_t scan_pair_bytes(int S, int E) { return (size_t)2 * S * 2 * E * 16 * sizeof(float); }
struct ScanPairLaunch {
    ScanDirection fwd, rev;
    const void* z;
    int64_t lddt;  int Rp;
    void* y;
    int S, L, E, dt;
    bool gate_each = false;
    float* ws;
    void* ysplit = nullptr;
    bool dt_split = false;
    int phases = 3;
};
hipError_t launch_scan_pair(const ScanPairLaunch& a, hipStream_t s);

constexpr int SCAN_BWD_CHUNK = 8;
struct ScanBwdLaunch {
    const void *u, *delta;
    const void* z = nullptr;  int64_t ldz = 0;
    const float *bc, *A, *Dskip, *dbias;
    const void* dout;
    void *du, *ddelta;
    void* dz = nullptr;
    float *dbc, *dA, *dD, *ddbias;
    void* scratch;
    int S, L, E, dt;
    bool reverse = false;
};
size_t scan_bwd_bytes(int S, int L, int E);
hipError_t launch_scan_bwd(const ScanBwdLaunch& a, hipStream_t s);

hipError_t launch_sum_partials(const float* part, int64_t P, float* out0, int n0, float* out1, int n1, hipStream_t s);

constexpr int CONV_BWD_SEG = 64;
struct ConvBwdLaunch {
    const void* x;  int64_t ldx;
    const float *w, *b;
    const void* dout;
    void* dx;
    float *dw, *db;
    void* scratch;
    int S, L, E, dt;
    bool reverse = false;
};
size_t conv_bwd_bytes(int S, int L, int E);
hipError_t launch_conv_bwd(const ConvBwdLaunch& a, hipStream_t s);

constexpr int NORM_BWD_ROWS = 16;
struct NormBwdLaunch {
    const void* x;
    const void* res_in = nullptr;
    const float* w;
    const void* dy;
    const void* dres_out = nullptr;
    void* dx;
    void* dres_in = nullptr;
    float* dw;
    void* scratch;
    int64_t rows;  int D;
    float eps;
    int dt, rdt;
};
size_t norm_bwd_bytes(int64_t rows, int D);
hipError_t launch_norm_bwd(const NormBwdLaunch& a, hipStream_t s);

struct LossHeadBwdLaunch {
    HeadInput in;
    const float* emb_f32;  const int32_t* comp8;
    const int32_t* labels;
    const float* loss_w = nullptr;
    int ignore_index;
    const float* dsum;
    const float* dnll = nullptr;
    void* dh = nullptr;
    void* dres = nullptr;
    float* dnorm_w = nullptr;
    float* demb = nullptr;
    void* scratch = nullptr;
};
size_t loss_head_bwd_bytes(int B, int L, int D);
hipError_t launch_loss_head_bwd(const LossHeadBwdLaunch& a, hipStream_t s);

constexpr int OPTIM_CHUNK = 4096;
struct AdamwLaunch {
    const void* table;  const int32_t* map;  int64_t chunks;
    void* state;
    float* part;
    float max_norm, grad_scale;
    float decay, b1, omb1, b2, omb2, step_size, bc2_sqrt, eps;
};
size_t optim_scratch_bytes(int64_t chunks);
hipError_t launch_adamw_step(const AdamwLaunch& a, hipStream_t s);
hipError_t launch_zero_grads(const void* table, const int32_t* map, int64_t chunks, hipStream_t s);

struct GatherRowsLaunch {
    const void* src;  void* out;
    int B, L, E;
    Positions pos;
    int dt;
    bool blocked = false;
};
hipError_t launch_gather_rows(const GatherRowsLaunch& g, hipStream_t s);
hipError_t launch_pack2d(const void* src, int src_dt, int64_t src_ld, void* dst, int dst_dt, int64_t dst_ld,
                         int rows, int cols, int dst_rows, int dst_cols, hipStream_t s);
hipError_t launch_pack_scale_cols(const void* src, int src_dt, int64_t src_ld, const float* scale, void* dst, int dst_dt,
                                  int64_t dst_ld, int rows, int cols, hipStream_t s);
hipError_t launch_embed_inproj_table(const void* emb, const void* Wf, void* tab, int V, int D, int N2, float eps, int dt, hipStream_t s);
hipError_t launch_embed_xz_gather(const int32_t* ids, const int32_t* comp8, const void* tab, void* x, void* z, int B, int L, int E, int dt,
                                  hipStream_t s);
hipError_t launch_pack_split_w(const void* src, int src_dt, int64_t src_ld, void* dst, int rows, int cols, hipStream_t s);
hipError_t launch_split_rows(const float* src, int64_t src_ld, void* dst, int64_t rows, int K, bool src_blocked, bool dst_blocked,
                             hipStream_t s);
hipError_t launch_pack_A(const void* A_log, int src_dt, float* A2, int64_t n, float scale, hipStream_t s);

}
```

### plantcaduceus_amd/csrc/pack.hip

```cpp
#include <mutex>
#include <set>
#include <utility>

#include "common.hpp"
#include "kernels.hpp"

namespace pcad {

template <typename SrcT, typename DstT>
__global__ __launch_bounds__(256) void pack2d_kernel(const SrcT* __restrict__ src, int64_t src_ld,
                                                     DstT* __restrict__ dst, int64_t dst_ld, int rows, int cols,
                                                     int dst_rows, int dst_cols) {
    const int64_t total = (int64_t)dst_rows * dst_cols;
    for (int64_t i = (int64_t)blockIdx.x * blockDim.x + threadIdx.x; i < total;
         i += (int64_t)gridDim.x * blockDim.x) {
        const int r = (int)(i / dst_cols), c = (int)(i - (int64_t)r * dst_cols);
        float v = 0.f;
        if (r < rows && c < cols) v = Elem<SrcT>::load(src + (int64_t)r * src_ld + c);
        Elem<DstT>::store(dst + (int64_t)r * dst_ld + c, v);
    }
}

hipError_t launch_pack2d(const void* src, int src_dt, int64_t src_ld, void* dst, int dst_dt, int64_t dst_ld, int rows,
                         int cols, int dst_rows, int dst_cols, hipStream_t s) {
    const int64_t total = (int64_t)dst_rows * dst_cols;
    if (total <= 0) return hipSuccess;
    int64_t nb = (total + 255) / 256;
    if (nb > 4096) nb = 4096;
    dim3 grid((unsigned)nb), block(256);
#define PCAD_PACK(ST, DT)                                                                                      \
    hipLaunchKernelGGL((pack2d_kernel<ST, DT>), grid, block, 0, s, (const ST*)src, src_ld, (DT*)dst, dst_ld, rows, \
                       cols, dst_rows, dst_cols)
    if (src_dt == F32 && dst_dt == F32) PCAD_PACK(float, float);
    else if (src_dt == F32 && dst_dt == BF16) PCAD_PACK(float, bf16_t);
    else if (src_dt == BF16 && dst_dt == F32) PCAD_PACK(bf16_t, float);
    else if (src_dt == BF16 && dst_dt == BF16) PCAD_PACK(bf16_t, bf16_t);
    else return hipErrorInvalidValue;
#undef PCAD_PACK
    return hipGetLastError();
}

template <typename SrcT>
__global__ __launch_bounds__(256) void pack_A_kernel(const SrcT* __restrict__ A_log, float* __restrict__ A2, int64_t n,
                                                     float scale) {
    const int64_t i = (int64_t)blockIdx.x * blockDim.x + threadIdx.x;
    if (i < n) A2[i] = -expf(Elem<SrcT>::load(A_log + i)) * scale;
}

template <typename SrcT, typename DstT>
__global__ __launch_bounds__(256) void pack_scale_cols_kernel(const SrcT* __restrict__ src, int64_t src_ld, const float* __restrict__ scale,
                                                              DstT* __restrict__ dst, int64_t dst_ld, int rows, int cols) {
    const int64_t total = (int64_t)rows * cols;
    for (int64_t i = (int64_t)blockIdx.x * blockDim.x + threadIdx.x; i < total; i += (int64_t)gridDim.x * blockDim.x) {
        const int r = (int)(i / cols), c = (int)(i - (int64_t)r * cols);
        Elem<DstT>::store(dst + (int64_t)r * dst_ld + c, Elem<SrcT>::load(src + (int64_t)r * src_ld + c) * scale[c]);
    }
}

hipError_t launch_pack_scale_cols(const void* src, int src_dt, int64_t src_ld, const float* scale, void* dst, int dst_dt,
                                  int64_t dst_ld, int rows, int cols, hipStream_t s) {
    const int64_t total = (int64_t)rows * cols;
    if (total <= 0) return hipSuccess;
    int64_t nb = (total + 255) / 256;
    if (nb > 4096) nb = 4096;
    dim3 grid((unsigned)nb), block(256);
#define PCAD_PSC(ST, DT) hipLaunchKernelGGL((pack_scale_cols_kernel<ST, DT>), grid, block, 0, s, (const ST*)src, src_ld, scale, (DT*)dst, dst_ld, rows, cols)
    if (src_dt == F32 && dst_dt == F32) PCAD_PSC(float, float);
    else if (src_dt == F32 && dst_dt == BF16) PCAD_PSC(float, bf16_t);
    else if (src_dt == BF16 && dst_dt == F32) PCAD_PSC(bf16_t, float);
    else PCAD_PSC(bf16_t, bf16_t);
#undef PCAD_PSC
    return hipGetLastError();
}

template <typename SrcT>
__global__ __launch_bounds__(256) void pack_split_w_kernel(const SrcT* __restrict__ src, int64_t src_ld, bf16_t* __restrict__ dst,
                                                           int rows, int cols) {
    const int64_t total = (int64_t)rows * cols;
    for (int64_t i = (int64_t)blockIdx.x * blockDim.x + threadIdx.x; i < total; i += (int64_t)gridDim.x * blockDim.x) {
        const int r = (int)(i / cols), c = (int)(i - (int64_t)r * cols);
        const float v = Elem<SrcT>::load(src + (int64_t)r * src_ld + c);
        const bf16_t hi = f32_to_bf16(v);
        const bf16_t lo = f32_to_bf16(v - bf16_to_f32(hi));
        bf16_t* d = dst + (int64_t)r * 2 * cols + c;
        d[0] = hi; d[cols] = lo;
    }
}

hipError_t launch_pack_split_w(const void* src, int src_dt, int64_t src_ld, void* dst, int rows, int cols, hipStream_t s) {
    const int64_t total = (int64_t)rows * cols;
    if (total <= 0) return hipSuccess;
    int64_t nb = (total + 255) / 256;
    if (nb > 4096) nb = 4096;
    if (src_dt == F32) hipLaunchKernelGGL(pack_split_w_kernel<float>, dim3((unsigned)nb), dim3(256), 0, s, (const float*)src, src_ld, (bf16_t*)dst, rows, cols);
    else hipLaunchKernelGGL(pack_split_w_kernel<bf16_t>, dim3((unsigned)nb), dim3(256), 0, s, (const bf16_t*)src, src_ld, (bf16_t*)dst, rows, cols);
    return hipGetLastError();
}

__global__ __launch_bounds__(256) void split_rows_kernel(const float* __restrict__ src, int64_t src_ld, bf16_t* __restrict__ dst, int64_t rows, int K,
                                                          int src_blocked, int dst_blocked) {
    const int nch = K >> 3;
    const int64_t total = rows * nch;
    for (int64_t i = (int64_t)blockIdx.x * blockDim.x + threadIdx.x; i < total; i += (int64_t)gridDim.x * blockDim.x) {
        const int64_t r = i / nch;
        const int c = (int)(i - r * nch) * 8;
        const float* sp = src_blocked ? reinterpret_cast<const float*>(reinterpret_cast<const char*>(src) + blocked_off(r, (int64_t)c * 4, (int64_t)K * 4 >> 7))
                                      : src + r * src_ld + c;
        float v[8], lo[8];
        load8<float>(sp, v);
#pragma unroll
        for (int k = 0; k < 8; ++k) lo[k] = v[k] - round_to_bf16(v[k]);
        auto at = [&](int col) -> bf16_t* {
            return dst_blocked ? reinterpret_cast<bf16_t*>(reinterpret_cast<char*>(dst) + blocked_off(r, (int64_t)col * 2, (int64_t)2 * K * 2 >> 7))
                               : dst + r * 2 * K + col;
        };
        store8<bf16_t>(at(c), v);
        store8<bf16_t>(at(K + c), lo);
    }
}

hipError_t launch_split_rows(const float* src, int64_t src_ld, void* dst, int64_t rows, int K, bool src_blocked, bool dst_blocked, hipStream_t s) {
    if (rows <= 0) return hipSuccess;
    if (K <= 0 || K % 64 || (!src_blocked && (src_ld < K || src_ld % 4)) || ((uintptr_t)src) % 16 || ((uintptr_t)dst) % 16) return hipErrorInvalidValue;
    const int64_t total = rows * (K >> 3);
    int64_t nb = (total + 255) / 256;
    if (nb > 65536) nb = 65536;
    hipLaunchKernelGGL(split_rows_kernel, dim3((unsigned)nb), dim3(256), 0, s, src, src_ld, (bf16_t*)dst, rows, K, (int)src_blocked, (int)dst_blocked);
    return hipGetLastError();
}

template <typename T>
__global__ __launch_bounds__(256) void embed_inproj_table_kernel(const T* __restrict__ emb, const T* __restrict__ Wf, T* __restrict__ tab,
                                                                 int D, int N2, float eps) {
    const int n = blockIdx.x * 256 + threadIdx.x, tok = blockIdx.y;
    if (n >= N2) return;
    const T* er = emb + (int64_t)tok * D;
    const T* wr = Wf + (int64_t)n * D;
    float acc = 0.f, ss = 0.f;
    for (int k = 0; k < D; ++k) {
        const float ev = Elem<T>::load(er + k);
        acc = __builtin_fmaf(ev, Elem<T>::load(wr + k), acc);
        ss = __builtin_fmaf(ev, ev, ss);
    }
    Elem<T>::store(tab + (int64_t)tok * N2 + n, acc * rsqrtf(ss / (float)D + eps));
}

hipError_t launch_embed_inproj_table(const void* emb, const void* Wf, void* tab, int V, int D, int N2, float eps, int dt, hipStream_t s) {
    dim3 grid((unsigned)((N2 + 255) / 256), (unsigned)V), block(256);
    if (dt == BF16) hipLaunchKernelGGL(embed_inproj_table_kernel<bf16_t>, grid, block, 0, s, (const bf16_t*)emb, (const bf16_t*)Wf, (bf16_t*)tab, D, N2, eps);
    else hipLaunchKernelGGL(embed_inproj_table_kernel<float>, grid, block, 0, s, (const float*)emb, (const float*)Wf, (float*)tab, D, N2, eps);
    return hipGetLastError();
}

template <typename T>
__global__ __launch_bounds__(256) void embed_xz_gather_kernel(const int32_t* __restrict__ ids, const int32_t* __restrict__ comp8,
                                                              const T* __restrict__ tab, T* __restrict__ x, T* __restrict__ z, int B, int L, int E) {
    const int lane = threadIdx.x & 63;
    const int64_t row = (int64_t)blockIdx.x * 4 + (threadIdx.x >> 6);
    if (row >= (int64_t)2 * B * L) return;
    const int s = (int)(row / L), t = (int)(row - (int64_t)s * L);
    int tok;
    if (s < B) tok = ids[(int64_t)s * L + t];
    else tok = comp8[ids[(int64_t)(s - B) * L + (L - 1 - t)] & 7];
    const char* src = reinterpret_cast<const char*>(tab + (int64_t)(tok & 7) * 2 * E);
    const int64_t rowb = (int64_t)E * sizeof(T), pieces = rowb >> 7;
    char* xb = reinterpret_cast<char*>(x);
    char* zb = reinterpret_cast<char*>(z);
    for (int64_t cb = (int64_t)lane * 16; cb < rowb; cb += 64 * 16) {
        const int64_t o = blocked_off(row, cb, pieces);
        *reinterpret_cast<u32x4*>(xb + o) = *reinterpret_cast<const u32x4*>(src + cb);
        *reinterpret_cast<u32x4*>(zb + o) = *reinterpret_cast<const u32x4*>(src + rowb + cb);
    }
}

hipError_t launch_embed_xz_gather(const int32_t* ids, const int32_t* comp8, const void* tab, void* x, void* z, int B, int L, int E, int dt,
                                  hipStream_t s) {
    const int64_t rows = (int64_t)2 * B * L;
    if (rows <= 0) return hipSuccess;
    if ((E * (dt == BF16 ? 2 : 4)) % 128) return hipErrorInvalidValue;
    dim3 grid((unsigned)((rows + 3) / 4)), block(256);
    if (dt == BF16) hipLaunchKernelGGL(embed_xz_gather_kernel<bf16_t>, grid, block, 0, s, ids, comp8, (const bf16_t*)tab, (bf16_t*)x, (bf16_t*)z, B, L, E);
    else hipLaunchKernelGGL(embed_xz_gather_kernel<float>, grid, block, 0, s, ids, comp8, (const float*)tab, (float*)x, (float*)z, B, L, E);
    return hipGetLastError();
}

hipError_t launch_pack_A(const void* A_log, int src_dt, float* A2, int64_t n, float scale, hipStream_t s) {
    if (n <= 0) return hipSuccess;
    dim3 grid((unsigned)((n + 255) / 256)), block(256);
    if (src_dt == F32) hipLaunchKernelGGL(pack_A_kernel<float>, grid, block, 0, s, (const float*)A_log, A2, n, scale);
    else hipLaunchKernelGGL(pack_A_kernel<bf16_t>, grid, block, 0, s, (const bf16_t*)A_log, A2, n, scale);
    return hipGetLastError();
}

template <typename T>
__global__ __launch_bounds__(256) void gather_rows_kernel(const T* __restrict__ src, T* __restrict__ out, int B, int L, int E,
                                                          Positions pos, int blocked) {
    const int P = pos.n;
    const int wave = (int)((blockIdx.x * blockDim.x + threadIdx.x) >> 6), lane = threadIdx.x & 63;
    if (wave >= 2 * B * P) return;
    const int strand = wave / P, q = wave - strand * P;
    int p = 0;
#pragma unroll
    for (int i = 0; i < 16; ++i)
        if (i == q) p = pos.p[i];
    const int64_t row = (int64_t)strand * L + (strand < B ? p : L - 1 - p);
    const int64_t rowb = (int64_t)E * sizeof(T);
    const char* sb = reinterpret_cast<const char*>(src);
    char* db = reinterpret_cast<char*>(out) + (int64_t)wave * rowb;
    for (int64_t cb = (int64_t)lane * 16; cb < rowb; cb += 64 * 16) {
        const int64_t so = blocked ? blocked_off(row, cb, rowb >> 7) : row * rowb + cb;
        *reinterpret_cast<u32x4*>(db + cb) = *reinterpret_cast<const u32x4*>(sb + so);
    }
}

hipError_t launch_gather_rows(const GatherRowsLaunch& g, hipStream_t s) {
    const int64_t rows = (int64_t)2 * g.B * g.pos.n;
    if (rows <= 0) return hipSuccess;
    const int esz = g.dt == BF16 ? 2 : 4;
    if ((g.E * esz) % 16 || (g.blocked && (g.E * esz) % 128)) return hipErrorInvalidValue;
    dim3 grid((unsigned)((rows + 3) / 4)), block(256);
    if (g.dt == BF16) hipLaunchKernelGGL(gather_rows_kernel<bf16_t>, grid, block, 0, s, (const bf16_t*)g.src, (bf16_t*)g.out, g.B, g.L, g.E, g.pos, (int)g.blocked);
    else hipLaunchKernelGGL(gather_rows_kernel<float>, grid, block, 0, s, (const float*)g.src, (float*)g.out, g.B, g.L, g.E, g.pos, (int)g.blocked);
    return hipGetLastError();
}

hipError_t ensure_dynamic_lds(const void* kernel, int bytes) {
    static std::mutex mu;
    static std::set<std::pair<int, const void*>> done;
    int dev = 0;
    hipError_t e = hipGetDevice(&dev);
    if (e != hipSuccess) return e;
    std::lock_guard<std::mutex> lock(mu);
    if (done.count({dev, kernel})) return hipSuccess;
    e = hipFuncSetAttribute(kernel, hipFuncAttributeMaxDynamicSharedMemorySize, bytes);
    if (e == hipSuccess) done.insert({dev, kernel});
    return e;
}

int device_cu_count() {
    static std::mutex mu;
    static int cus[64] = {0};
    int dev = 0;
    if (hipGetDevice(&dev) != hipSuccess || dev < 0 || dev >= 64) return 256;
    std::lock_guard<std::mutex> lock(mu);
    if (!cus[dev]) {
        hipDeviceProp_t prop;
        cus[dev] = hipGetDeviceProperties(&prop, dev) == hipSuccess && prop.multiProcessorCount > 0 ? prop.multiProcessorCount : 256;
    }
    return cus[dev];
}

}
```

### plantcaduceus_amd/csrc/pcad_internal.hpp

```cpp
#pragma once
#include <hip/hip_runtime.h>
#include <vector>
#include "../../include/pcad.h"
#include "kernels.hpp"

namespace pcad {
int fail(int code, const char* fmt, ...);

#define HIP_TRY(expr)                                                                             \
    do {                                                                                          \
        hipError_t _e = (expr);                                                                   \
        if (_e != hipSuccess) return fail(PCAD_ERR_HIP, "%s: %s", #expr, hipGetErrorString(_e)); \
    } while (0)

inline size_t align_up(size_t v, size_t a = 256) { return (v + a - 1) / a * a; }

struct DirWeights {
    float *conv_w, *conv_b;
    void* Wx;
    void* Wx_s;
    void* Wdt;
    void* Wdt_s;
    float *dt_bias, *A2, *Dskip;
};
struct LayerWeights {
    float* convw;
    float* norm_w;
    void* W_in;
    void* W_in_f;
    void* W_out;
    void* W_out_p;
    void* W_in_s;
    void* W_out_s;
    void *W_in_r, *W_out_r, *W_in_s_r, *W_out_s_r;
    DirWeights dir[2];
};
}

struct pcad_engine {
    pcad_config cfg;
    int D, E, N, R, Rp, XP, V, nl;
    int esz;
    int rdt;
    int chunk;
    int64_t chunk_rows;
    bool gate_once;
    bool convx;
    bool xzsplit;
    bool blocked;
    bool segments = true;
    bool shortcut = true;
    int ref_order = 0;
    int norm_fold = -1;
    int rep_class = -1, rep_count = 1;
    bool poison = false;
    bool bound = false;
    int64_t ws_limit = 0;
    bool f32_split = false;
    bool split_packed = false;
    bool untied = false;
    bool untied_packed = false;
    bool fold_packed = false;
    int32_t* status = nullptr;
    std::vector<pcad::LayerWeights> layers;
    void* xz_tab0 = nullptr;
    void* emb = nullptr;
    float* emb_f32 = nullptr;
    float* normf_w = nullptr;
    int32_t* comp = nullptr;
    bool prof = false;
    int prof_stride = 1;
    int64_t prof_seen[PCAD_NUM_KERNEL_CLASSES] = {0};
    std::vector<std::pair<hipEvent_t, hipEvent_t>> prof_ev[PCAD_NUM_KERNEL_CLASSES];
    std::vector<hipEvent_t> prof_pool;
    double prof_ms[PCAD_NUM_KERNEL_CLASSES] = {0};
    int64_t prof_n[PCAD_NUM_KERNEL_CLASSES] = {0};
};

namespace pcad {
bool fold_wanted(const pcad_engine* e);
bool split_wanted(const pcad_engine* e);
struct SmallForms {
    int G = 1;
    bool pair = false;
    int ksplit = 1;
};
SmallForms small_forms(const pcad_engine* e, int B, int L);
struct Workspace {
    void *res, *u, *h, *xz, *zb, *xc[2], *dtl[2], *y;
    void *xz2, *zb2;
    void* ys;
    float* bc[2];
    float *rstd, *ssq;
    float* seg;
    float* pair;
    float* cxp;
    size_t bytes;
};
Workspace carve_workspace(const pcad_engine* e, void* base, int Bc, int L, int Bpol);
int chunk_for(const pcad_engine* e, int B, int L);
hipEvent_t prof_event(pcad_engine* e);
constexpr size_t kProfCap = 1 << 16;
struct ProfScope {
    pcad_engine* e; int cls; hipStream_t s; hipEvent_t a = nullptr, b = nullptr;
    ProfScope(pcad_engine* e_, int cls_, hipStream_t s_) : e(e_), cls(cls_), s(s_) {
        if (e->prof && (e->prof_seen[cls]++ % e->prof_stride) == 0 && e->prof_ev[cls].size() < kProfCap) {
            a = prof_event(e); b = prof_event(e);
            if (a) (void)hipEventRecord(a, s);
        }
    }
    ~ProfScope() {
        if (a && b) { (void)hipEventRecord(b, s); e->prof_ev[cls].push_back({a, b}); }
    }
};

int positions_arg(const char* who, const int32_t* positions, int P, int L, Positions* pos);
int probs_cols_arg(const char* who, const int32_t* cols, int vocab, ProbCols* out);

}
```

### plantcaduceus_amd/csrc/scan.hip

```cpp
#include <array>
#include <cstdlib>
#include <initializer_list>
#include <type_traits>

#include "common.hpp"
#include "kernels.hpp"

namespace pcad {

typedef float f2 __attribute__((ext_vector_type(2)));
typedef float f32x16 __attribute__((ext_vector_type(16)));
typedef __bf16 bf16x8_t __attribute__((ext_vector_type(8)));

constexpr int NSTATE = 16;
constexpr int TB = 32;
#ifndef PCAD_SCAN_CH
#define PCAD_SCAN_CH 4
#endif
#ifndef PCAD_SCAN_OCC
#define PCAD_SCAN_OCC 4
#endif
#ifndef PCAD_SCAN_OCC96
#define PCAD_SCAN_OCC96 PCAD_SCAN_OCC
#endif
constexpr int CH = PCAD_SCAN_CH;

__device__ __forceinline__ float exp2_hw(float x) { return __builtin_amdgcn_exp2f(x); }

typedef __attribute__((address_space(8))) void* rsrc_t;
__device__ __forceinline__ auto make_rsrc(const void* base, uint32_t bytes) {
    return __builtin_amdgcn_make_buffer_rsrc(const_cast<void*>(base), 0, (int)bytes, 0x00020000);
}
constexpr int SCAN_AUX = 2;
template <typename T> struct BufIO;
template <> struct BufIO<bf16_t> {
    template <typename R> static __device__ __forceinline__ bf16_t load(R r, int voff, uint32_t soff) {
        return (bf16_t)__builtin_amdgcn_raw_buffer_load_b16(r, voff, (int)soff, SCAN_AUX);
    }
    template <typename R> static __device__ __forceinline__ void store(bf16_t v, R r, int voff, uint32_t soff) {
        __builtin_amdgcn_raw_buffer_store_b16(v, r, voff, (int)soff, SCAN_AUX);
    }
};
template <> struct BufIO<float> {
    template <typename R> static __device__ __forceinline__ float load(R r, int voff, uint32_t soff) {
        return __uint_as_float(__builtin_amdgcn_raw_buffer_load_b32(r, voff, (int)soff, SCAN_AUX));
    }
    template <typename R> static __device__ __forceinline__ void store(float v, R r, int voff, uint32_t soff) {
        __builtin_amdgcn_raw_buffer_store_b32(__float_as_uint(v), r, voff, (int)soff, SCAN_AUX);
    }
};

template <typename T> struct DeltaTile;

template <> struct DeltaTile<bf16_t> {
    static __device__ __forceinline__ void run(const bf16_t* __restrict__ dtl, int64_t lddt, int64_t row_base, int t0,
                                               int L, const bf16_t* __restrict__ Wdt, int c0, int Rp, int lane,
                                               f32x16& acc0, f32x16& acc1) {
        const int tr = max(0, min(t0 + (lane & 31), L - 1));
        const bf16_t* arow = dtl + (row_base + tr) * lddt + (lane >> 5) * 8;
        const bf16_t* b0 = Wdt + (int64_t)(c0 + (lane & 31)) * Rp + (lane >> 5) * 8;
        const bf16_t* b1 = b0 + (int64_t)32 * Rp;
#pragma unroll 4
        for (int k = 0; k < Rp; k += 16) {
            const u32x4 a = *reinterpret_cast<const u32x4*>(arow + k);
            const u32x4 w0 = *reinterpret_cast<const u32x4*>(b0 + k);
            const u32x4 w1 = *reinterpret_cast<const u32x4*>(b1 + k);
            acc0 = __builtin_amdgcn_mfma_f32_32x32x16_bf16(__builtin_bit_cast(bf16x8_t, a),
                                                           __builtin_bit_cast(bf16x8_t, w0), acc0, 0, 0, 0);
            acc1 = __builtin_amdgcn_mfma_f32_32x32x16_bf16(__builtin_bit_cast(bf16x8_t, a),
                                                           __builtin_bit_cast(bf16x8_t, w1), acc1, 0, 0, 0);
        }
    }
};

template <int RP> struct DeltaPre { u32x4 a[RP / 16]; };
template <int RP>
__device__ __forceinline__ DeltaPre<RP> delta_prefetch(const bf16_t* __restrict__ dtl, int64_t lddt, int64_t row_base,
                                                       int t0, int L, int lane) {
    const int tr = max(0, min(t0 + (lane & 31), L - 1));
    const bf16_t* arow = dtl + (row_base + tr) * lddt + (lane >> 5) * 8;
    DeltaPre<RP> p;
#pragma unroll
    for (int k = 0; k < RP / 16; ++k) p.a[k] = *reinterpret_cast<const u32x4*>(arow + k * 16);
    return p;
}
template <int RP>
__device__ __forceinline__ void delta_run_pre(const DeltaPre<RP>& p, const bf16_t* __restrict__ Wdt, int c0, int lane,
                                              f32x16& acc0, f32x16& acc1) {
    const bf16_t* b0 = Wdt + (int64_t)(c0 + (lane & 31)) * RP + (lane >> 5) * 8;
    const bf16_t* b1 = b0 + (int64_t)32 * RP;
#pragma unroll
    for (int k = 0; k < RP / 16; ++k) {
        const u32x4 w0 = *reinterpret_cast<const u32x4*>(b0 + k * 16);
        const u32x4 w1 = *reinterpret_cast<const u32x4*>(b1 + k * 16);
        acc0 = __builtin_amdgcn_mfma_f32_32x32x16_bf16(__builtin_bit_cast(bf16x8_t, p.a[k]),
                                                       __builtin_bit_cast(bf16x8_t, w0), acc0, 0, 0, 0);
        acc1 = __builtin_amdgcn_mfma_f32_32x32x16_bf16(__builtin_bit_cast(bf16x8_t, p.a[k]),
                                                       __builtin_bit_cast(bf16x8_t, w1), acc1, 0, 0, 0);
    }
}

template <> struct DeltaTile<float> {
    static __device__ __forceinline__ void run(const float* __restrict__ dtl, int64_t lddt, int64_t row_base, int t0,
                                               int L, const float* __restrict__ Wdt, int c0, int Rp, int lane,
                                               f32x16& acc0, f32x16& acc1) {
        const int tr = max(0, min(t0 + (lane & 31), L - 1));
        const int kh = (lane >> 5) * (Rp >> 1);
        const float* arow = dtl + (row_base + tr) * lddt + kh;
        const float* b0 = Wdt + (int64_t)(c0 + (lane & 31)) * Rp + kh;
        const float* b1 = b0 + (int64_t)32 * Rp;
        for (int k = 0; k < (Rp >> 1); k += 4) {
            const f32x4 a = *reinterpret_cast<const f32x4*>(arow + k);
            const f32x4 w0 = *reinterpret_cast<const f32x4*>(b0 + k);
            const f32x4 w1 = *reinterpret_cast<const f32x4*>(b1 + k);
#pragma unroll
            for (int j = 0; j < 4; ++j) {
                acc0 = __builtin_amdgcn_mfma_f32_32x32x2f32(a[j], w0[j], acc0, 0, 0, 0);
                acc1 = __builtin_amdgcn_mfma_f32_32x32x2f32(a[j], w1[j], acc1, 0, 0, 0);
            }
        }
    }
};

struct DeltaTileSplit {
    static __device__ __forceinline__ void run64(const bf16_t* __restrict__ arow, const bf16_t* __restrict__ b0, const bf16_t* __restrict__ b1,
                                                 f32x16& acc0, f32x16& acc1) {
        constexpr int NK = 4, RP = 64;
        u32x4 ah[NK], al[NK], w0[NK], w1[NK];
#pragma unroll
        for (int k = 0; k < NK; ++k) {
            ah[k] = *reinterpret_cast<const u32x4*>(arow + k * 16);
            al[k] = *reinterpret_cast<const u32x4*>(arow + RP + k * 16);
            w0[k] = *reinterpret_cast<const u32x4*>(b0 + k * 16);
            w1[k] = *reinterpret_cast<const u32x4*>(b1 + k * 16);
        }
        auto mm = [&](const u32x4& a, const u32x4& x0, const u32x4& x1) {
            acc0 = __builtin_amdgcn_mfma_f32_32x32x16_bf16(__builtin_bit_cast(bf16x8_t, a), __builtin_bit_cast(bf16x8_t, x0), acc0, 0, 0, 0);
            acc1 = __builtin_amdgcn_mfma_f32_32x32x16_bf16(__builtin_bit_cast(bf16x8_t, a), __builtin_bit_cast(bf16x8_t, x1), acc1, 0, 0, 0);
        };
#pragma unroll
        for (int k = 0; k < NK; ++k) mm(ah[k], w0[k], w1[k]);
#pragma unroll
        for (int k = 0; k < NK; ++k) mm(al[k], w0[k], w1[k]);
#pragma unroll
        for (int k = 0; k < NK; ++k) {
            w0[k] = *reinterpret_cast<const u32x4*>(b0 + RP + k * 16);
            w1[k] = *reinterpret_cast<const u32x4*>(b1 + RP + k * 16);
        }
#pragma unroll
        for (int k = 0; k < NK; ++k) mm(ah[k], w0[k], w1[k]);
    }
    static __device__ __forceinline__ void run(const bf16_t* __restrict__ dtl, int64_t lddt, int64_t row_base, int t0,
                                               int L, const bf16_t* __restrict__ Wdt, int c0, int Rp, int lane,
                                               f32x16& acc0, f32x16& acc1) {
        const int tr = max(0, min(t0 + (lane & 31), L - 1));
        const bf16_t* arow = dtl + (row_base + tr) * lddt + (lane >> 5) * 8;
        const bf16_t* b0 = Wdt + (int64_t)(c0 + (lane & 31)) * 2 * Rp + (lane >> 5) * 8;
        const bf16_t* b1 = b0 + (int64_t)32 * 2 * Rp;
#ifndef PCAD_SCAN_TILE_GENERIC
        if (Rp == 64) { run64(arow, b0, b1, acc0, acc1); return; }
#endif
#pragma unroll
        for (int part = 0; part < 3; ++part) {
            const bf16_t* ap = arow + (part == 1 ? Rp : 0);
            const int wo = part == 2 ? Rp : 0;
#pragma unroll 4
            for (int k = 0; k < Rp; k += 16) {
                const u32x4 a = *reinterpret_cast<const u32x4*>(ap + k);
                const u32x4 w0 = *reinterpret_cast<const u32x4*>(b0 + wo + k);
                const u32x4 w1 = *reinterpret_cast<const u32x4*>(b1 + wo + k);
                acc0 = __builtin_amdgcn_mfma_f32_32x32x16_bf16(__builtin_bit_cast(bf16x8_t, a),
                                                               __builtin_bit_cast(bf16x8_t, w0), acc0, 0, 0, 0);
                acc1 = __builtin_amdgcn_mfma_f32_32x32x16_bf16(__builtin_bit_cast(bf16x8_t, a),
                                                               __builtin_bit_cast(bf16x8_t, w1), acc1, 0, 0, 0);
            }
        }
    }
};

template <typename T, bool REV, int ACC, bool HASZ, bool FUSED, int PRE, bool BLK8, int SEG = 0, bool ZB = false, bool SPLITY = false>
__device__ __forceinline__ void scan_body(float (*dvs)[64], const int block_id, const int num_blocks,
                                          const T* __restrict__ u, const T* __restrict__ z, int64_t ldz,
                                          const T* __restrict__ dsrc, int64_t ldd,
                                          const T* __restrict__ Wdt, int Rp,
                                          const float* __restrict__ bc,
                                          const float* __restrict__ A2, float a_scale,
                                          const float* __restrict__ Dskip, const float* __restrict__ dbias,
                                          const T* yin, T* y, int L, int E, int uyb, int zblk, int G, int seg_blocks,
                                          float* __restrict__ seg_state, int Lw, bf16_t* __restrict__ ysplit, int dts) {
    const int lane = threadIdx.x;
    const int ncb = E >> 6;
    const int nss = num_blocks / ncb;
    int ss, cb;
    {
        const int b = block_id, full = (nss & ~7) * ncb;
        if (b < full) { const int j = b >> 3, q = j / ncb; ss = q * 8 + (b & 7); cb = j - q * ncb; }
        else { const int r = b - full, q = r / ncb; ss = (nss & ~7) + q; cb = r - q * ncb; }
    }
    const int c0 = cb * 64;
    const int c = c0 + lane;
    constexpr bool PAIR = SEG == 3 || SEG == 4;
    const int strand = PAIR ? ss : (SEG ? ss / G : ss);
    const int seg = PAIR ? (SEG == 4 ? 1 : 0) : (SEG ? ss - strand * G : 0);
    const int nstrands = PAIR ? nss : (SEG ? nss / G : nss);
    const int64_t row0 = (int64_t)strand * L;

    f2 a2p[NSTATE / 2], hp[NSTATE / 2];
#pragma unroll
    for (int p = 0; p < NSTATE / 2; p += 2) {
        const f32x4 v = *reinterpret_cast<const f32x4*>(A2 + (int64_t)c * NSTATE + 2 * p);
        a2p[p] = f2{v[0] * a_scale, v[1] * a_scale};
        a2p[p + 1] = f2{v[2] * a_scale, v[3] * a_scale};
    }
    float* __restrict__ seg_h = seg_state + (((int64_t)strand * G + seg) * E + c) * NSTATE;
    if constexpr (SEG == 2 || SEG == 4) {
#pragma unroll
        for (int p = 0; p < NSTATE / 2; p += 2) {
            const f32x4 v = *reinterpret_cast<const f32x4*>(seg_h + 2 * p);
            hp[p] = f2{v[0], v[1]};
            hp[p + 1] = f2{v[2], v[3]};
        }
    } else {
#pragma unroll
        for (int p = 0; p < NSTATE / 2; ++p) hp[p] = f2{0.f, 0.f};
    }
    float dsum = 0.f;
    const float dsk = Dskip[c];
    const float db = dbias[c];

    const int nblk = (Lw + TB - 1) / TB;
    const uint32_t esz = (uint32_t)sizeof(T);
    const uint32_t rowE = (uint32_t)E * esz, rowZ = (uint32_t)ldz * esz, rowD = (uint32_t)ldd * esz;
    const uint32_t pieces = rowE >> 7;
    const uint32_t tot_rows = ((uint32_t)nstrands * (uint32_t)L + 7u) & ~7u;
    const bool blk = BLK8 || uyb;
    const auto u_r = blk ? make_rsrc(u, tot_rows * rowE) : make_rsrc(u + row0 * E + c0, (uint32_t)L * rowE);
    const auto y_r = blk ? make_rsrc(y, tot_rows * rowE) : make_rsrc(y + row0 * E + c0, (uint32_t)L * rowE);
    const bool zb_ = ZB || (HASZ && blk && zblk);
    const auto z_r = zb_ ? make_rsrc(z, tot_rows * rowE) : make_rsrc(HASZ ? z + row0 * ldz + c0 : u, (uint32_t)L * rowZ);
    const auto d_r = make_rsrc(FUSED ? u : dsrc + row0 * ldd + c0, (uint32_t)L * rowD);
    const float* __restrict__ bc_s = bc + row0 * (2 * NSTATE);
    const int voff = lane * (int)esz;
    const int voff_uy = blk ? (int)((((uint32_t)voff >> 7) << 10) + ((uint32_t)voff & 127u)) : voff;
    const uint32_t c0b = (uint32_t)c0 * esz;
    auto off_uy = [&](uint32_t t) -> uint32_t {
        if (blk) {
            const uint32_t r = (uint32_t)row0 + t;
            return (((r >> 3) * pieces + (c0b >> 7)) << 10) + ((r & 7u) << 7);
        }
        return t * rowE;
    };
    auto uy_soff = [&](int s0, int i) -> uint32_t {
        if constexpr (BLK8) {
            const int slo = min(REV ? s0 + CH - 1 : s0, L - 1);
            return off_uy((uint32_t)(REV ? (L - 1 - slo) : slo));
        } else {
            const int sc = min(s0 + i, L - 1);
            return off_uy((uint32_t)(REV ? (L - 1 - sc) : sc));
        }
    };
    auto uy_voff = [&](int i) -> int { return BLK8 ? voff_uy + 128 * (REV ? CH - 1 - i : i) : voff_uy; };
    const uint32_t ys_pieces = (2u * (uint32_t)E * 2u) >> 7, ys_half = ((uint32_t)E >> 6) << 10;
    const auto ys_r = make_rsrc(SPLITY ? (const void*)ysplit : (const void*)u, SPLITY ? tot_rows * 2u * (uint32_t)E * 2u : 4u);
    auto ys_soff = [&](int s0) -> uint32_t {
        const int slo = min(REV ? s0 + CH - 1 : s0, L - 1);
        const uint32_t r = (uint32_t)row0 + (uint32_t)(REV ? (L - 1 - slo) : slo);
        return (((r >> 3) * ys_pieces + ((uint32_t)c0 >> 6)) << 10) + ((r & 7u) << 7);
    };
    auto ys_voff = [&](int i) -> int { return lane * 2 + 128 * (REV ? CH - 1 - i : i); };

    T ub[CH], zb[CH], yb[CH], dr[CH];
    auto tclamp = [&](int s) { const int sc = min(s, L - 1); return REV ? (L - 1 - sc) : sc; };
    auto load_chunk = [&](int s0, T (&uu)[CH], T (&zz)[CH], T (&yy)[CH], T (&dd)[CH]) {
#pragma unroll
        for (int i = 0; i < CH; ++i) {
            const uint32_t t = (uint32_t)tclamp(s0 + i);
#ifdef PCAD_SCAN_HOT
            const uint32_t so = uy_soff(s0, i) & 0xffffu;
#else
            const uint32_t so = uy_soff(s0, i);
#endif
            uu[i] = BufIO<T>::load(u_r, uy_voff(i), so);
            if constexpr (HASZ && ZB) zz[i] = BufIO<T>::load(z_r, uy_voff(i), so);
            else if constexpr (HASZ) zz[i] = zb_ ? BufIO<T>::load(z_r, uy_voff(i), so) : BufIO<T>::load(z_r, voff, t * rowZ);
            if constexpr (ACC != 0) yy[i] = BufIO<T>::load(y_r, uy_voff(i), so);
            if constexpr (!FUSED) dd[i] = BufIO<T>::load(d_r, voff, t * rowD);
        }
    };
    const int b_begin = SEG ? seg * seg_blocks : 0;
    const int s_first = b_begin * TB;
    load_chunk(s_first, ub, zb, yb, dr);

    f2 bcc[NSTATE];
    auto load_bc = [&](int s, f2 (&dst)[NSTATE]) {
        const f2* __restrict__ r = reinterpret_cast<const f2*>(bc_s + (uint32_t)tclamp(s) * (uint32_t)(2 * NSTATE));
#pragma unroll
        for (int p = 0; p < NSTATE; ++p) dst[p] = r[p];
    };
    load_bc(s_first, bcc);

    float dv_cur = 0.f;
    auto step = [&](int s, int i, const float* dvp, float uv, float zv, float yprev, T draw) -> float {
        f2 bcn[NSTATE];
        load_bc(s + 1, bcn);
        float dv, dv_next = 0.f;
        if constexpr (FUSED) {
            dv = dv_cur;
            dv_next = dvp[(REV ? CH - 1 - i : i + 2) * 64];
        } else {
            dv = softplus(Elem<T>::to_f32(draw) + db);
        }
        const float du = dv * uv;
        const f2 dv2 = {dv, dv}, du2 = {du, du};
        f2 yacc = {ACC == 2 ? __builtin_fmaf(dsk, uv, yprev) : dsk * uv, 0.f};
        if constexpr (SEG == 1) dsum += dv;
#pragma unroll
        for (int p = 0; p < NSTATE / 2; ++p) {
            const f2 e0 = dv2 * a2p[p];
            const f2 a0 = {exp2_hw(e0[0]), exp2_hw(e0[1])};
            hp[p] = a0 * hp[p] + du2 * bcc[p];
            if constexpr (SEG != 1) yacc = hp[p] * bcc[NSTATE / 2 + p] + yacc;
        }
        float yv = 0.f;
        if constexpr (SEG != 1) {
            yv = yacc[0] + yacc[1];
            if constexpr (HASZ) yv *= silu(zv);
            if constexpr (ACC == 1) {
                if constexpr (std::is_same<T, float>::value) asm volatile("" : "+v"(yv));
                yv = Elem<T>::round(yv) + yprev;
            }
        }
#pragma unroll
        for (int p = 0; p < NSTATE; ++p) bcc[p] = bcn[p];
        dv_cur = dv_next;
        return yv;
    };

    DeltaPre<PRE ? PRE : 16> pre;
    if constexpr (PRE != 0) pre = delta_prefetch<PRE>((const bf16_t*)dsrc, ldd, row0, REV ? (L - (b_begin + 1) * TB) : b_begin * TB, L, lane);

    float pfb0 = 0.f, pfb1 = 0.f;
    const int b_end = SEG ? min(nblk, b_begin + seg_blocks) : nblk;
    for (int b = b_begin; b < b_end; ++b) {
        const int tb0 = REV ? (L - (b + 1) * TB) : b * TB;
#ifndef PCAD_SCAN_NOPF
        if constexpr (FUSED) {
            asm volatile("" ::"v"(pfb0), "v"(pfb1));
            const int tbn = max(0, min(REV ? (L - (b + 2) * TB) : (b + 1) * TB, L - 1));
            {
                const int lim = L * (2 * NSTATE * 4) - 4;
                const char* pb = reinterpret_cast<const char*>(bc_s);
                pfb0 = *reinterpret_cast<const float*>(pb + min(tbn * (2 * NSTATE * 4) + lane * 32, lim));
                pfb1 = *reinterpret_cast<const float*>(pb + min(tbn * (2 * NSTATE * 4) + (64 + lane) * 32, lim));
            }
        }
#endif
        if constexpr (FUSED) {
            f32x16 acc0, acc1;
#pragma unroll
            for (int i = 0; i < 16; ++i) { acc0[i] = 0.f; acc1[i] = 0.f; }
            if constexpr (PRE != 0) {
                delta_run_pre<PRE>(pre, (const bf16_t*)Wdt, c0, lane, acc0, acc1);
                pre = delta_prefetch<PRE>((const bf16_t*)dsrc, ldd, row0, REV ? (L - (b + 2) * TB) : (b + 1) * TB, L, lane);
            } else if constexpr (std::is_same<T, float>::value) {
                if (dts) DeltaTileSplit::run(reinterpret_cast<const bf16_t*>(dsrc), ldd, row0, tb0, L, reinterpret_cast<const bf16_t*>(Wdt), c0, Rp, lane, acc0, acc1);
                else DeltaTile<T>::run(dsrc, ldd, row0, tb0, L, Wdt, c0, Rp, lane, acc0, acc1);
            } else {
                DeltaTile<T>::run(dsrc, ldd, row0, tb0, L, Wdt, c0, Rp, lane, acc0, acc1);
            }
#pragma unroll
            for (int r = 0; r < 16; ++r) {
                const auto sw = __builtin_amdgcn_permlane32_swap(__float_as_uint(acc0[r]), __float_as_uint(acc1[r]),
                                                                 false, false);
                const int tt = (r & 3) + 8 * (r >> 2);
                const f2 dl = softplus2(Elem<T>::round2(f2{__uint_as_float(sw[0]), __uint_as_float(sw[1])}) + f2{db, db});
                dvs[tt + 1][lane] = dl[0];
                dvs[tt + 5][lane] = dl[1];
            }
        }
        const int s_begin = b * TB;
        const int s_end = min(Lw, s_begin + TB);
        if constexpr (FUSED) dv_cur = dvs[REV ? TB : 1][lane];
        auto dv_base = [&](int s0) -> const float* { return &dvs[REV ? TB - CH - (s0 - s_begin) : (s0 - s_begin)][lane]; };
        auto run_step = [&](int s, int i, const float* dvp, uint32_t oy, int vy, T uraw, T zraw, T yraw, T draw, uint32_t oys) {
            const float yv0 = step(s, i, dvp, Elem<T>::to_f32(uraw), HASZ ? Elem<T>::to_f32(zraw) : 0.f,
                                   ACC != 0 ? Elem<T>::to_f32(yraw) : 0.f, draw);
            if constexpr (SPLITY && SEG != 1) {
                float yq = yv0;
                asm volatile("" : "+v"(yq));
                const float yv = yq;
                const uint32_t pk = pack_bf16x2(yv, 0.f);
                const bf16_t hi = (bf16_t)(pk & 0xffffu);
                const bf16_t lo = f32_to_bf16(yv - bf16lo_to_f32(pk));
#ifdef PCAD_SCAN_HOTSTORE
                BufIO<bf16_t>::store(hi, ys_r, ys_voff(i), oys & 0xffffu);
                BufIO<bf16_t>::store(lo, ys_r, ys_voff(i), (oys & 0xffffu) + ys_half);
            } else if constexpr (SEG != 1) BufIO<T>::store(Elem<T>::from_f32(yv0), y_r, vy, oy & 0xffffu);
#else
                BufIO<bf16_t>::store(hi, ys_r, ys_voff(i), oys);
                BufIO<bf16_t>::store(lo, ys_r, ys_voff(i), oys + ys_half);
            } else if constexpr (SEG != 1) BufIO<T>::store(Elem<T>::from_f32(yv0), y_r, vy, oy);
#endif
        };
        auto run_chunk = [&](int s0, T (&uu)[CH], T (&zz)[CH], T (&yy)[CH], T (&dd)[CH]) {
            const float* dvp = dv_base(s0);
            const uint32_t oys = SPLITY ? ys_soff(s0) : 0u;
#pragma unroll
            for (int i = 0; i < CH; ++i) run_step(s0 + i, i, dvp, uy_soff(s0, i), uy_voff(i), uu[i], zz[i], yy[i], dd[i], oys);
        };
        int s0 = s_begin;
        T un[CH], zn[CH], yn[CH], dn[CH];
        for (; s0 + 2 * CH <= s_end; s0 += 2 * CH) {
            load_chunk(s0 + CH, un, zn, yn, dn);
            run_chunk(s0, ub, zb, yb, dr);
            load_chunk(s0 + 2 * CH, ub, zb, yb, dr);
            run_chunk(s0 + CH, un, zn, yn, dn);
        }
        if (s0 + CH <= s_end) {
            load_chunk(s0 + CH, un, zn, yn, dn);
            run_chunk(s0, ub, zb, yb, dr);
#pragma unroll
            for (int i = 0; i < CH; ++i) { ub[i] = un[i]; zb[i] = zn[i]; yb[i] = yn[i]; dr[i] = dn[i]; }
            s0 += CH;
        }
        if (s0 < s_end) {
            const float* dvp = dv_base(s0);
#pragma unroll
            for (int i = 0; i < CH - 1; ++i)
                if (s0 + i < s_end) run_step(s0 + i, i, dvp, uy_soff(s0, i), uy_voff(i), ub[i], zb[i], yb[i], dr[i], SPLITY ? ys_soff(s0) : 0u);
        }
    }
    if constexpr (SEG == 1) {
#pragma unroll
        for (int p = 0; p < NSTATE / 2; p += 2)
            *reinterpret_cast<f32x4*>(seg_h + 2 * p) = f32x4{hp[p][0], hp[p][1], hp[p + 1][0], hp[p + 1][1]};
        seg_state[(int64_t)nstrands * G * E * NSTATE + ((int64_t)strand * G + seg) * E + c] = dsum;
    }
    if constexpr (SEG == 3) {
        float* __restrict__ nxt = seg_h + (int64_t)E * NSTATE;
#pragma unroll
        for (int p = 0; p < NSTATE / 2; p += 2)
            *reinterpret_cast<f32x4*>(nxt + 2 * p) = f32x4{hp[p][0], hp[p][1], hp[p + 1][0], hp[p + 1][1]};
    }
}

template <typename T, bool REV, int ACC, bool HASZ, bool FUSED, int PRE, bool BLK8, int SEG = 0, bool ZB = false, bool SPLITY = false>
__global__ __launch_bounds__(64, PRE == 96 ? PCAD_SCAN_OCC96 : PCAD_SCAN_OCC) void scan_kernel(const T* __restrict__ u, const T* __restrict__ z, int64_t ldz,
                                                  const T* __restrict__ dsrc, int64_t ldd,
                                                  const T* __restrict__ Wdt, int Rp,
                                                  const float* __restrict__ bc,
                                                  const float* __restrict__ A2, float a_scale,
                                                  const float* __restrict__ Dskip, const float* __restrict__ dbias,
                                                  const T* yin, T* y, int L, int E, int uyb, int zblk, int G, int seg_blocks,
                                                  float* __restrict__ seg_state, int Lw, bf16_t* __restrict__ ysplit, int dts) {
    __shared__ float dvs[TB + 2][64];
    scan_body<T, REV, ACC, HASZ, FUSED, PRE, BLK8, SEG, ZB, SPLITY>(dvs, (int)blockIdx.x, (int)gridDim.x, u, z, ldz, dsrc, ldd, Wdt, Rp, bc, A2, a_scale,
                                                                    Dskip, dbias, yin, y, L, E, uyb, zblk, G, seg_blocks, seg_state, Lw, ysplit, dts);
}

template <typename T, int ACC, bool HASZ, int PRE, int PHASE, bool SPLITY>
__global__ __launch_bounds__(64, PRE == 96 ? PCAD_SCAN_OCC96 : PCAD_SCAN_OCC) void scan_pair_kernel(
    const T* __restrict__ u0, const T* __restrict__ dsrc0, const T* __restrict__ Wdt0, const float* __restrict__ bc0, const float* __restrict__ A2_0,
    const float* __restrict__ Dskip0, const float* __restrict__ dbias0, float* __restrict__ seg0,
    const T* __restrict__ u1, const T* __restrict__ dsrc1, const T* __restrict__ Wdt1, const float* __restrict__ bc1, const float* __restrict__ A2_1,
    const float* __restrict__ Dskip1, const float* __restrict__ dbias1, float* __restrict__ seg1,
    const T* __restrict__ z, int64_t ldd, int Rp, float a_scale, T* y, int L, int E, int seg_blocks, bf16_t* __restrict__ ysplit, int dts) {
    __shared__ float dvs[TB + 2][64];
    const int half = (int)gridDim.x >> 1;
    if ((int)blockIdx.x < half)
        scan_body<T, false, ACC, HASZ, true, PRE, true, PHASE, HASZ, SPLITY>(dvs, (int)blockIdx.x, half, u0, z, (int64_t)E, dsrc0, ldd, Wdt0, Rp, bc0, A2_0, a_scale,
                                                                             Dskip0, dbias0, y, y, L, E, 1, 1, 2, seg_blocks, seg0, L, ysplit, dts);
    else
        scan_body<T, true, ACC, HASZ, true, PRE, true, PHASE, HASZ, SPLITY>(dvs, (int)blockIdx.x - half, half, u1, z, (int64_t)E, dsrc1, ldd, Wdt1, Rp, bc1, A2_1, a_scale,
                                                                            Dskip1, dbias1, y, y, L, E, 1, 1, 2, seg_blocks, seg1, L, ysplit, dts);
}

__global__ __launch_bounds__(256) void scan_carry_kernel(float* __restrict__ seg_state, const float* __restrict__ A2, float a_scale,
                                                         int S, int G, int E) {
    const int64_t i = (int64_t)blockIdx.x * blockDim.x + threadIdx.x;
    if (i >= (int64_t)S * E) return;
    const int strand = (int)(i / E), c = (int)(i - (int64_t)strand * E);
    const float* dsum = seg_state + (int64_t)S * G * E * NSTATE;
    float a[NSTATE], h[NSTATE];
#pragma unroll
    for (int n = 0; n < NSTATE; ++n) { a[n] = A2[(int64_t)c * NSTATE + n] * a_scale; h[n] = 0.f; }
    for (int g = 0; g < G; ++g) {
        float* hs = seg_state + (((int64_t)strand * G + g) * E + c) * NSTATE;
        const float ds = dsum[((int64_t)strand * G + g) * E + c];
#pragma unroll
        for (int n = 0; n < NSTATE; ++n) {
            const float hend = hs[n];
            hs[n] = h[n];
            h[n] = exp2_hw(a[n] * ds) * h[n] + hend;
        }
    }
}

struct ScanForm {
    bool rev; int acc; bool has_z; int seg; bool splity;
    bool operator==(const ScanForm& o) const { return rev == o.rev && acc == o.acc && has_z == o.has_z && seg == o.seg && splity == o.splity; }
};
template <typename Row, size_t N, typename Form>
static auto find_kernel(const Row (&rows)[N], const Form& form) -> decltype(rows[0].kernel) {
    for (const Row& r : rows)
        if (r.form == form) return r.kernel;
    return nullptr;
}

template <typename T, bool FUSED, int PRE, bool BLK8, bool ZB>
struct ScanFamily {
    using Kernel = decltype(&scan_kernel<T, false, 0, false, FUSED, PRE, BLK8>);
    struct Row { ScanForm form; Kernel kernel; };
    template <bool REV, int ACC, bool HZ, int SEG = 0, bool SPLITY = false>
    static Row row() { return {{REV, ACC, HZ, SEG, SPLITY}, scan_kernel<T, REV, ACC, HZ, FUSED, PRE, BLK8, SEG, ZB && HZ, SPLITY>}; }

    static int slot(const ScanForm& f) { return (((f.seg * 2 + f.rev) * 3 + f.acc) * 2 + f.has_z) * 2 + f.splity; }
    static Kernel kernel(const ScanForm& f) {
        static const std::array<Kernel, 72> table = [] {
            std::array<Kernel, 72> t{};
            auto add = [&t](std::initializer_list<Row> rows) { for (const Row& r : rows) t[slot(r.form)] = r.kernel; };
            add({row<false, 0, false>(), row<false, 0, true>(), row<false, 1, false>(), row<false, 1, true>(), row<false, 2, true>(),
                 row<true, 0, false>(),  row<true, 0, true>(),  row<true, 1, false>(),  row<true, 1, true>(),  row<true, 2, true>()});
            if constexpr (FUSED)
                add({row<false, 0, false, 1>(), row<true, 0, false, 1>(),
                     row<false, 0, false, 2>(), row<false, 0, true, 2>(), row<true, 0, true, 2>(), row<true, 1, true, 2>(), row<true, 2, true, 2>()});
            if constexpr (std::is_same<T, float>::value && FUSED && BLK8 && ZB)
                add({row<true, 1, true, 0, true>(), row<true, 2, true, 0, true>()});
            return t;
        }();
        return f.seg >= 0 && f.seg <= 2 && f.acc >= 0 && f.acc <= 2 ? table[slot(f)] : nullptr;
    }
};

enum class ScanFamilyId { BF16_ENGINE64, BF16_ENGINE96, BF16_BLK8, BF16_PRE64, BF16_FUSED, BF16_DELTA, F32_ENGINE, F32_FUSED, F32_DELTA };

struct ScanPlan {
    ScanFamilyId family;
    ScanForm form;
    int G = 1, seg_blocks = 0;
};

static hipError_t scan_plan(const ScanLaunch& a, ScanPlan& p) {
    const bool fused = a.delta == nullptr;
    const bool blk8 = a.uy_blocked && a.L % 8 == 0;
    if (a.dt == BF16) {
        static const bool nopre96 = dev_env("PCAD_SCAN_NOPRE96") != nullptr;
        const bool pre = fused && a.lddt % 8 == 0;
        if (pre && a.Rp == 64 && blk8 && a.z_blocked) p.family = ScanFamilyId::BF16_ENGINE64;
        else if (!nopre96 && pre && a.Rp == 96 && blk8 && a.z_blocked) p.family = ScanFamilyId::BF16_ENGINE96;
        else if (pre && a.Rp == 64 && blk8) p.family = ScanFamilyId::BF16_BLK8;
        else if (pre && a.Rp == 64) p.family = ScanFamilyId::BF16_PRE64;
        else p.family = fused ? ScanFamilyId::BF16_FUSED : ScanFamilyId::BF16_DELTA;
    } else {
        static const bool f32_generic = dev_env("PCAD_SCAN_F32_GENERIC") != nullptr;
        if (!f32_generic && fused && blk8 && a.z_blocked) p.family = ScanFamilyId::F32_ENGINE;
        else p.family = fused ? ScanFamilyId::F32_FUSED : ScanFamilyId::F32_DELTA;
    }
    const int Sp = a.policy_S > 0 ? a.policy_S : a.S;
    const bool hz = a.z != nullptr, reverse = a.reverse;
    const int accumulate = a.accumulate;
    if (a.ysplit != nullptr) {
        const bool seg = a.seg_ws && scan_segments(Sp, a.L, a.E, nullptr) > 1;
        if (p.family != ScanFamilyId::F32_ENGINE || !reverse || !hz || (accumulate != 1 && accumulate != 2) || seg || (a.walk_len > 0 && a.walk_len < a.L))
            return hipErrorInvalidValue;
        p.form = {true, accumulate, true, 0, true};
        return hipSuccess;
    }
    if (fused) {
        int sb = 0;
        const int G = a.seg_ws ? scan_segments(Sp, a.L, a.E, &sb) : 1;
        const bool combo = (!reverse && accumulate == 0) || (reverse && hz && (accumulate == 0 || accumulate == 1 || accumulate == 2));
        if (G > 1 && combo) {
            p.form = {reverse, accumulate, hz, 2, false};
            p.G = G;
            p.seg_blocks = sb;
            return hipSuccess;
        }
    }
    if (accumulate == 2 && !hz) return hipErrorInvalidValue;
    p.form = {reverse, accumulate == 2 ? 2 : (accumulate ? 1 : 0), hz, 0, false};
    return hipSuccess;
}

template <typename T, bool FUSED, int PRE = 0, bool BLK8 = false, bool ZB = false>
static hipError_t launch_scan_t(const ScanLaunch& a, const ScanPlan& p, hipStream_t s) {
    using Family = ScanFamily<T, FUSED, PRE, BLK8, ZB>;
    const ScanDirection& d = a.dir;
    const T* dsrc = (const T*)(FUSED ? d.dt_low : a.delta);
    const int64_t ldd = FUSED ? a.lddt : a.E;
    const T* Wdt = FUSED ? (const T*)d.Wdt : nullptr;
    const int Rp = FUSED ? a.Rp : 0, dts = a.dt_split ? 1 : 0, S = a.S, L = a.L, E = a.E;
    auto launch = [&](const ScanForm& f, const T* z, int G, int seg_blocks, float* seg_ws, int walk, bf16_t* ysplit) {
        const typename Family::Kernel k = Family::kernel(f);
        if (!k) return hipErrorInvalidValue;
        hipLaunchKernelGGL(k, dim3((unsigned)((int64_t)(E / 64) * S * G)), dim3(64), 0, s, (const T*)d.u, z, a.ldz, dsrc, ldd, Wdt, Rp, d.bc, d.A2, a.a_scale,
                           d.Dskip, d.dbias, (const T*)a.y, (T*)a.y, L, E, (int)a.uy_blocked, (int)a.z_blocked, G, seg_blocks, seg_ws, walk, ysplit, dts);
        return hipSuccess;
    };
    if (p.G > 1) {
        if (hipError_t e = launch({p.form.rev, 0, false, 1, false}, nullptr, p.G, p.seg_blocks, a.seg_ws, L, nullptr)) return e;
        hipLaunchKernelGGL(scan_carry_kernel, dim3((unsigned)(((int64_t)S * E + 255) / 256)), dim3(256), 0, s, a.seg_ws, d.A2, a.a_scale, S, p.G, E);
        if (hipError_t e = launch(p.form, (const T*)a.z, p.G, p.seg_blocks, a.seg_ws, L, nullptr)) return e;
    } else {
        const int walk = !p.form.splity && a.walk_len > 0 && a.walk_len < L ? a.walk_len : L;
        if (hipError_t e = launch(p.form, (const T*)a.z, 1, 0, nullptr, walk, p.form.splity ? (bf16_t*)a.ysplit : nullptr)) return e;
    }
    return hipGetLastError();
}

struct ScanPairForm {
    int acc; bool has_z; int phase; bool splity;
    bool operator==(const ScanPairForm& o) const { return acc == o.acc && has_z == o.has_z && phase == o.phase && splity == o.splity; }
};

template <typename T, int PRE>
struct ScanPairFamily {
    using Kernel = decltype(&scan_pair_kernel<T, 0, false, PRE, 3, false>);
    struct Row { ScanPairForm form; Kernel kernel; };
    template <int ACC, bool HZ, int PHASE, bool SPLITY = false>
    static Row row() { return {{ACC, HZ, PHASE, SPLITY}, scan_pair_kernel<T, ACC, HZ, PRE, PHASE, SPLITY>}; }
    static Kernel kernel(const ScanPairForm& f) {
        static const Row rows[] = {row<0, false, 3>(), row<0, true, 3>(), row<1, true, 4>(), row<2, true, 4>()};
        if (Kernel k = find_kernel(rows, f)) return k;
        if constexpr (std::is_same<T, float>::value) {
            static const Row splity[] = {row<1, true, 4, true>(), row<2, true, 4, true>()};
            return find_kernel(splity, f);
        }
        return nullptr;
    }
};

template <typename T, int PRE>
static hipError_t launch_scan_pair_t(const ScanPairLaunch& a, hipStream_t s) {
    const int sb = (a.L / TB) / 2;
    float* seg0 = a.ws;
    float* seg1 = a.ws + (size_t)a.S * 2 * a.E * NSTATE;
    const ScanDirection &f = a.fwd, &r = a.rev;
    auto launch = [&](const ScanPairForm& form) {
        const typename ScanPairFamily<T, PRE>::Kernel k = ScanPairFamily<T, PRE>::kernel(form);
        if (!k) return hipErrorInvalidValue;
        hipLaunchKernelGGL(k, dim3((unsigned)((int64_t)2 * a.S * (a.E / 64))), dim3(64), 0, s,
                           (const T*)f.u, (const T*)f.dt_low, (const T*)f.Wdt, f.bc, f.A2, f.Dskip, f.dbias, seg0,
                           (const T*)r.u, (const T*)r.dt_low, (const T*)r.Wdt, r.bc, r.A2, r.Dskip, r.dbias, seg1,
                           (const T*)a.z, a.lddt, a.Rp, 1.0f, (T*)a.y, a.L, a.E, sb, (bf16_t*)a.ysplit, a.dt_split ? 1 : 0);
        return hipSuccess;
    };
    if (a.phases & 1)
        if (hipError_t e = launch({0, a.gate_each, 3, false})) return e;
    if (!(a.phases & 2)) return hipGetLastError();
    if (hipError_t e = launch({a.gate_each ? 1 : 2, true, 4, a.ysplit != nullptr})) return e;
    return hipGetLastError();
}

hipError_t launch_scan_pair(const ScanPairLaunch& a, hipStream_t s) {
    const int S = a.S, L = a.L, E = a.E, Rp = a.Rp, dt = a.dt;
    const int64_t lddt = a.lddt;
    if (S <= 0 || L <= 0) return hipSuccess;
    if (!a.ws || !a.z || E % 64 || L % (2 * TB) || Rp <= 0 || Rp % 32) return hipErrorInvalidValue;
    const int esz = dt == BF16 ? 2 : 4;
    if ((E * esz) % 128 || ((int64_t)S * L + 7) / 8 * 8 * E * esz >= ((int64_t)1 << 32)) return hipErrorInvalidValue;
    if ((int64_t)L * E * 4 >= ((int64_t)1 << 31)) return hipErrorInvalidValue;
    if (a.dt_split && !(dt == F32 && Rp <= 96 && lddt % 8 == 0 && lddt >= 2 * Rp)) return hipErrorInvalidValue;
    if (a.ysplit && !(dt == F32 && ((int64_t)S * L + 7) / 8 * 8 * 2 * E * 2 < ((int64_t)1 << 32))) return hipErrorInvalidValue;
    if (dt == BF16) {
        if (lddt % 8) return hipErrorInvalidValue;
        if (Rp == 64) return launch_scan_pair_t<bf16_t, 64>(a, s);
        if (Rp == 96) return launch_scan_pair_t<bf16_t, 96>(a, s);
        return hipErrorInvalidValue;
    }
    return launch_scan_pair_t<float, 0>(a, s);
}

hipError_t launch_scan(const ScanLaunch& a, hipStream_t s) {
    const int S = a.S, L = a.L, E = a.E, Rp = a.Rp, dt = a.dt;
    const int64_t lddt = a.lddt, ldz = a.ldz;
    if (a.z_blocked && !a.uy_blocked) return hipErrorInvalidValue;
    if (a.dt_split && !(dt == F32 && a.delta == nullptr && Rp % 32 == 0 && Rp <= 96 && lddt % 8 == 0 && lddt >= 2 * Rp)) return hipErrorInvalidValue;
    if (a.ysplit && !(dt == F32 && a.delta == nullptr && a.uy_blocked && a.z_blocked && L % 8 == 0 && ((int64_t)S * L + 7) / 8 * 8 * 2 * E * 2 < ((int64_t)1 << 32)))
        return hipErrorInvalidValue;
    if (S <= 0 || L <= 0) return hipSuccess;
    if (E % 64) return hipErrorInvalidValue;
    if ((int64_t)L * (ldz > E ? ldz : E) * 4 >= ((int64_t)1 << 31)) return hipErrorInvalidValue;
    if (a.uy_blocked && (((int64_t)S * L + 7) / 8 * 8 * E * (dt == BF16 ? 2 : 4) >= ((int64_t)1 << 32) || (E * (dt == BF16 ? 2 : 4)) % 128))
        return hipErrorInvalidValue;
    if (a.delta == nullptr && (!a.dir.dt_low || !a.dir.Wdt || Rp <= 0 || Rp % 32)) return hipErrorInvalidValue;
    ScanPlan p;
    if (hipError_t e = scan_plan(a, p)) return e;
    switch (p.family) {
    case ScanFamilyId::BF16_ENGINE64: return launch_scan_t<bf16_t, true, 64, true, true>(a, p, s);
    case ScanFamilyId::BF16_ENGINE96: return launch_scan_t<bf16_t, true, 96, true, true>(a, p, s);
    case ScanFamilyId::BF16_BLK8:     return launch_scan_t<bf16_t, true, 64, true>(a, p, s);
    case ScanFamilyId::BF16_PRE64:    return launch_scan_t<bf16_t, true, 64>(a, p, s);
    case ScanFamilyId::BF16_FUSED:    return launch_scan_t<bf16_t, true>(a, p, s);
    case ScanFamilyId::BF16_DELTA:    return launch_scan_t<bf16_t, false>(a, p, s);
    case ScanFamilyId::F32_ENGINE:    return launch_scan_t<float, true, 0, true, true>(a, p, s);
    case ScanFamilyId::F32_FUSED:     return launch_scan_t<float, true>(a, p, s);
    case ScanFamilyId::F32_DELTA:     return launch_scan_t<float, false>(a, p, s);
    }
    return hipErrorInvalidValue;
}

}
```

Measured before the change: 1210 sequences/s.

## Trim last layer to gathered positions: sparse z projection and sparse scan output

For the last layer when only a few output positions are needed, the in-projection computes only the x half for all rows. The z half is computed by gathering the wanted rows, running a small GEMM and scattering them back into the blocked layout. The scan gains a SPARSE variant that updates state at every step but loads z/y and emits output only at the wanted positions. This avoids half of the last layer's in-proj GEMM and most of the scan's output work, at the cost of extra gather/scatter launches, more kernel instantiations and workspace-fit conditions.

```diff
diff --git a/plantcaduceus_amd/csrc/api.hip b/plantcaduceus_amd/csrc/api.hip
--- a/plantcaduceus_amd/csrc/api.hip
+++ b/plantcaduceus_amd/csrc/api.hip
@@ -276,6 +276,8 @@
         h->segments = value != 0;
     } else if (k == "last_layer_shortcut") {
         h->shortcut = value != 0;
+    } else if (k == "last_block_trim") {
+        h->trim = value != 0;
     } else {
         return fail(PCAD_ERR_INVALID, "pcad_set_option: unknown option '%s'", key);
     }
diff --git a/plantcaduceus_amd/csrc/forward.hip b/plantcaduceus_amd/csrc/forward.hip
--- a/plantcaduceus_amd/csrc/forward.hip
+++ b/plantcaduceus_amd/csrc/forward.hip
@@ -37,6 +37,7 @@
     bool lay_inter, strict;
     int depth;
     int walk_len;
+    bool trim;
     SmallForms forms;
     bool tab0;
     int Q;
@@ -68,6 +69,17 @@
         const int need = (pmax + 1 > L - pmin) ? pmax + 1 : L - pmin;
         pl.walk_len = (need + 7) / 8 * 8;
         if (pl.walk_len > L) pl.walk_len = L;
+    }
+    pl.trim = false;
+    if (pl.walk_len > 0 && e->trim && rq.head == Head::lm && !truncated && !pl.untied && !pl.strict && e->xzsplit && e->blocked && pl.forms.G == 1 &&
+        (!pl.fold || E % 256 == 0)) {
+        const size_t arow = pl.fold ? (size_t)fold_padded_width(D) * e->esz : pl.sp ? (size_t)2 * D * 2 : (size_t)D * e->esz;
+        auto fits = [&](int Bc) {
+            const size_t n = (size_t)2 * Bc * P;
+            return align_up(n * arow) + n * E * 4 <= ((size_t)2 * Bc * L + 7) / 8 * 8 * E * e->esz;
+        };
+        const int tail = B - (pl.nchunks - 1) * pl.chunk;
+        pl.trim = fits(pl.chunk) && fits(tail);
     }
     static const bool tab0 = dev_env("PCAD_NO_TAB0") == nullptr;
     pl.tab0 = tab0;
@@ -122,6 +134,32 @@
         if (e->xzsplit) return launch_gemm_nt_two(g, {.C1 = x, .C2 = z, .nsplit = E, .out_blocked = true}, s);
         return launch_gemm_nt(g, {.C = x, .ldc = 2 * E, .out_dt = dt}, s);
     }
+    bool trimmed(int li) const { return pl.trim && last_short(li); }
+    bool sparse_scan(int li) const { return trimmed(li) && L % 8 == 0 && (dt == F32 || Rp == 64 || Rp == 96); }
+    hipError_t in_proj_x(const Lane& c, const LayerWeights& W, int64_t rows) const {
+        if (pl.fold)
+            return launch_gemm_nt_two({.A = c.w.u, .lda = Dp, .W = W.W_in_f, .ldw = D, .M = rows, .N = E, .K = D, .dt = dt},
+                                      {.C1 = c.w.xz, .C2 = nullptr, .nsplit = E, .out_blocked = true, .rscale = c.w.rstd}, s);
+        if (pl.sp)
+            return launch_gemm_nt_two({.A = c.w.u, .lda = 2 * D, .W = W.W_in_s, .ldw = 2 * D, .M = rows, .N = E, .K = 3 * D, .dt = BF16, .ksplit = D / 64},
+                                      {.C1 = c.w.xz, .C2 = nullptr, .nsplit = E, .out_blocked = true, .out_dt = F32}, s);
+        return launch_gemm_nt_two({.A = c.w.u, .lda = D, .W = W.W_in, .ldw = D, .M = rows, .N = E, .K = D, .dt = dt},
+                                  {.C1 = c.w.xz, .C2 = nullptr, .nsplit = E, .out_blocked = true}, s);
+    }
+    int in_proj_z(Lane& c, const LayerWeights& W) const {
+        const int64_t n = (int64_t)2 * c.Bc * P;
+        const int adt = pl.sp ? (int)BF16 : dt;
+        const int64_t lda = pl.fold ? Dp : pl.sp ? 2 * D : D, ldw = pl.sp ? 2 * D : D;
+        const size_t aesz = adt == BF16 ? 2 : 4;
+        void* Ag = c.w.y;
+        float* Zg = (float*)((char*)c.w.y + align_up((size_t)n * lda * aesz));
+        const void* Wz = (const char*)(pl.fold ? W.W_in_f : pl.sp ? W.W_in_s : W.W_in) + (size_t)E * ldw * aesz;
+        HIP_TRY(launch_gather_rows({.src = c.w.u, .out = Ag, .B = c.Bc, .L = L, .E = (int)lda, .pos = pos, .dt = adt}, s));
+        if (pl.sp) HIP_TRY(launch_gemm_nt({.A = Ag, .lda = lda, .W = Wz, .ldw = ldw, .M = n, .N = E, .K = 3 * D, .dt = BF16, .ksplit = D / 64}, {.C = Zg, .ldc = E, .out_dt = F32}, s));
+        else HIP_TRY(launch_gemm_nt({.A = Ag, .lda = lda, .W = Wz, .ldw = ldw, .M = n, .N = E, .K = D, .dt = dt}, {.C = Zg, .ldc = E, .out_dt = F32}, s));
+        HIP_TRY(launch_scatter_rows({.src = Zg, .out = c.w.zb, .B = c.Bc, .L = L, .E = E, .pos = pos, .dt = dt, .rscale = pl.fold ? c.w.rstd : nullptr}, s));
+        return PCAD_OK;
+    }
     int64_t ldxz() const { return e->xzsplit ? E : 2 * E; }
     ScanDirection scan_dir(const Lane& c, const LayerWeights& W, int d, bool dts) const {
         const DirWeights& dw = W.dir[d];
@@ -209,10 +247,15 @@
         } else
         for (int rep = 0; rep < reps(PCAD_K_GEMM_IN); ++rep)
         { ProfScope ps(e, PCAD_K_GEMM_IN, s);
-        if (pl.fold)
+        if (trimmed(li)) HIP_TRY(in_proj_x(c, W, rows));
+        else if (pl.fold)
             HIP_TRY(launch_gemm_nt_two({.A = c.w.u, .lda = Dp, .W = W.W_in_f, .ldw = D, .M = rows, .N = 2 * E, .K = D, .dt = dt},
                                        {.C1 = c.w.xz, .C2 = c.w.zb, .nsplit = E, .out_blocked = true, .rscale = c.w.rstd}, s));
         else HIP_TRY(in_proj(c, W, rows, 0, c.w.xz, c.w.zb)); }
+        if (trimmed(li) && !(pl.fold && li == 0 && pl.tab0)) {
+            ProfScope ps(e, PCAD_K_HEAD, s);
+            if (int rc = in_proj_z(c, W)) return rc;
+        }
         if (convx_fused(rows)) for (int rep = 0; rep < reps(PCAD_K_CONV); ++rep) {
             ProfScope ps(e, PCAD_K_CONV, s);
             ConvxLaunch cx{.x = c.w.xz, .convw = W.convw, .S = S, .L = L, .E = E, .dt = dt, .Rp = Rp,
@@ -263,6 +306,7 @@
             sc.accumulate = strict ? 0 : (d == 1 ? (e->gate_once ? 2 : 1) : 0);
             sc.walk_len = last_short(li) ? pl.walk_len : 0;
             sc.ysplit = d == 1 && ys_from_scan ? c.w.ys : nullptr;
+            if (sparse_scan(li)) sc.out_rows = pos;
             HIP_TRY(launch_scan(sc, s));
         }
         return PCAD_OK;
diff --git a/plantcaduceus_amd/csrc/gemm.hip b/plantcaduceus_amd/csrc/gemm.hip
--- a/plantcaduceus_amd/csrc/gemm.hip
+++ b/plantcaduceus_amd/csrc/gemm.hip
@@ -1004,9 +1004,10 @@
     const int esz = dt == BF16 ? 2 : 4;
     const int out_dt = o.out_dt < 0 ? dt : o.out_dt;
     const int osz = out_dt == BF16 ? 2 : 4;
-    if (K <= 0 || (K * esz) % ROWB || nsplit % 16 || N % 16 || nsplit <= 0 || nsplit >= N || g.a_blocked) return hipErrorInvalidValue;
+    if (K <= 0 || (K * esz) % ROWB || nsplit % 16 || N % 16 || nsplit <= 0 || nsplit > N || g.a_blocked) return hipErrorInvalidValue;
     if ((g.lda * esz) % 16 || (g.ldw * esz) % 16 || ((uintptr_t)g.A) % 16 || ((uintptr_t)g.W) % 16) return hipErrorInvalidValue;
-    if (((uintptr_t)o.C1) % 16 || ((uintptr_t)o.C2) % 16) return hipErrorInvalidValue;
+    void* const C2 = nsplit == N ? o.C1 : o.C2;
+    if (((uintptr_t)o.C1) % 16 || ((uintptr_t)C2) % 16) return hipErrorInvalidValue;
     if (o.out_blocked && ((nsplit * osz) % 128 || ((N - nsplit) * osz) % 128)) return hipErrorInvalidValue;
     if (out_dt != dt) {
         if (dt != BF16 || out_dt != F32 || o.rscale) return hipErrorInvalidValue;
@@ -1014,7 +1015,7 @@
     } else if (ksplit) {
         return hipErrorInvalidValue;
     }
-    return launch_gemm256(g, out_dt, {.C = o.C1, .ldc = nsplit, .C2 = o.C2, .nsplit = nsplit, .out_blocked = o.out_blocked,
+    return launch_gemm256(g, out_dt, {.C = o.C1, .ldc = nsplit, .C2 = C2, .nsplit = nsplit, .out_blocked = o.out_blocked,
                                       .epi_kind = o.rscale ? EPI_SCALE : EPI_NONE, .epi = {o.rscale, nullptr, nullptr}}, s);
 }
 
diff --git a/plantcaduceus_amd/csrc/kernels.hpp b/plantcaduceus_amd/csrc/kernels.hpp
--- a/plantcaduceus_amd/csrc/kernels.hpp
+++ b/plantcaduceus_amd/csrc/kernels.hpp
@@ -201,6 +201,7 @@
     void* ysplit = nullptr;
     bool dt_split = false;
     int policy_S = 0;
+    Positions out_rows = {};
 };
 hipError_t launch_scan(const ScanLaunch& a, hipStream_t s);
 
@@ -332,6 +333,14 @@
     bool blocked = false;
 };
 hipError_t launch_gather_rows(const GatherRowsLaunch& g, hipStream_t s);
+struct ScatterRowsLaunch {
+    const float* src;  void* out;
+    int B, L, E;
+    Positions pos;
+    int dt;
+    const float* rscale = nullptr;
+};
+hipError_t launch_scatter_rows(const ScatterRowsLaunch& g, hipStream_t s);
 hipError_t launch_pack2d(const void* src, int src_dt, int64_t src_ld, void* dst, int dst_dt, int64_t dst_ld,
                          int rows, int cols, int dst_rows, int dst_cols, hipStream_t s);
 hipError_t launch_pack_scale_cols(const void* src, int src_dt, int64_t src_ld, const float* scale, void* dst, int dst_dt,
diff --git a/plantcaduceus_amd/csrc/pack.hip b/plantcaduceus_amd/csrc/pack.hip
--- a/plantcaduceus_amd/csrc/pack.hip
+++ b/plantcaduceus_amd/csrc/pack.hip
@@ -224,6 +224,43 @@
     return hipGetLastError();
 }
 
+template <typename T>
+__global__ __launch_bounds__(256) void scatter_rows_kernel(const float* __restrict__ src, T* __restrict__ out, int B, int L, int E, Positions pos,
+                                                           const float* __restrict__ rscale) {
+    const int P = pos.n;
+    const int wave = (int)((blockIdx.x * blockDim.x + threadIdx.x) >> 6), lane = threadIdx.x & 63;
+    if (wave >= 2 * B * P) return;
+    const int strand = wave / P, q = wave - strand * P;
+    int p = 0;
+#pragma unroll
+    for (int i = 0; i < 16; ++i)
+        if (i == q) p = pos.p[i];
+    const int64_t row = (int64_t)strand * L + (strand < B ? p : L - 1 - p);
+    const float rs = rscale ? rscale[row] : 1.0f;
+    const float* sr = src + (int64_t)wave * E;
+    char* ob = reinterpret_cast<char*>(out);
+    for (int c = lane * 8; c < E; c += 64 * 8) {
+        float v[8];
+        load8<float>(sr + c, v);
+        if (rscale) {
+#pragma unroll
+            for (int k = 0; k < 8; ++k) v[k] *= rs;
+        }
+        store8<T>(reinterpret_cast<T*>(ob + blocked_off(row, (int64_t)c * sizeof(T), ((int64_t)E * sizeof(T)) >> 7)), v);
+    }
+}
+
+hipError_t launch_scatter_rows(const ScatterRowsLaunch& g, hipStream_t s) {
+    const int64_t rows = (int64_t)2 * g.B * g.pos.n;
+    if (rows <= 0) return hipSuccess;
+    const int esz = g.dt == BF16 ? 2 : 4;
+    if ((g.E * esz) % 128 || ((uintptr_t)g.src) % 16 || ((uintptr_t)g.out) % 16) return hipErrorInvalidValue;
+    dim3 grid((unsigned)((rows + 3) / 4)), block(256);
+    if (g.dt == BF16) hipLaunchKernelGGL(scatter_rows_kernel<bf16_t>, grid, block, 0, s, g.src, (bf16_t*)g.out, g.B, g.L, g.E, g.pos, g.rscale);
+    else hipLaunchKernelGGL(scatter_rows_kernel<float>, grid, block, 0, s, g.src, (float*)g.out, g.B, g.L, g.E, g.pos, g.rscale);
+    return hipGetLastError();
+}
+
 hipError_t ensure_dynamic_lds(const void* kernel, int bytes) {
     static std::mutex mu;
     static std::set<std::pair<int, const void*>> done;
diff --git a/plantcaduceus_amd/csrc/pcad_internal.hpp b/plantcaduceus_amd/csrc/pcad_internal.hpp
--- a/plantcaduceus_amd/csrc/pcad_internal.hpp
+++ b/plantcaduceus_amd/csrc/pcad_internal.hpp
@@ -50,6 +50,7 @@
     bool blocked;
     bool segments = true;
     bool shortcut = true;
+    bool trim = true;
     int ref_order = 0;
     int norm_fold = -1;
     int rep_class = -1, rep_count = 1;
diff --git a/plantcaduceus_amd/csrc/scan.hip b/plantcaduceus_amd/csrc/scan.hip
--- a/plantcaduceus_amd/csrc/scan.hip
+++ b/plantcaduceus_amd/csrc/scan.hip
@@ -178,7 +178,7 @@
     }
 };
 
-template <typename T, bool REV, int ACC, bool HASZ, bool FUSED, int PRE, bool BLK8, int SEG = 0, bool ZB = false, bool SPLITY = false>
+template <typename T, bool REV, int ACC, bool HASZ, bool FUSED, int PRE, bool BLK8, int SEG = 0, bool ZB = false, bool SPLITY = false, bool SPARSE = false>
 __device__ __forceinline__ void scan_body(float (*dvs)[64], const int block_id, const int num_blocks,
                                           const T* __restrict__ u, const T* __restrict__ z, int64_t ldz,
                                           const T* __restrict__ dsrc, int64_t ldd,
@@ -187,7 +187,8 @@
                                           const float* __restrict__ A2, float a_scale,
                                           const float* __restrict__ Dskip, const float* __restrict__ dbias,
                                           const T* yin, T* y, int L, int E, int uyb, int zblk, int G, int seg_blocks,
-                                          float* __restrict__ seg_state, int Lw, bf16_t* __restrict__ ysplit, int dts) {
+                                          float* __restrict__ seg_state, int Lw, bf16_t* __restrict__ ysplit, int dts,
+                                          const Positions want = {}, const int want_half = 0) {
     const int lane = threadIdx.x;
     const int ncb = E >> 6;
     const int nss = num_blocks / ncb;
@@ -281,9 +282,11 @@
             const uint32_t so = uy_soff(s0, i);
 #endif
             uu[i] = BufIO<T>::load(u_r, uy_voff(i), so);
+            if constexpr (!SPARSE) {
             if constexpr (HASZ && ZB) zz[i] = BufIO<T>::load(z_r, uy_voff(i), so);
             else if constexpr (HASZ) zz[i] = zb_ ? BufIO<T>::load(z_r, uy_voff(i), so) : BufIO<T>::load(z_r, voff, t * rowZ);
             if constexpr (ACC != 0) yy[i] = BufIO<T>::load(y_r, uy_voff(i), so);
+            }
             if constexpr (!FUSED) dd[i] = BufIO<T>::load(d_r, voff, t * rowD);
         }
     };
@@ -300,7 +303,8 @@
     load_bc(s_first, bcc);
 
     float dv_cur = 0.f;
-    auto step = [&](int s, int i, const float* dvp, float uv, float zv, float yprev, T draw) -> float {
+    auto step = [&](int s, int i, const float* dvp, float uv, float zv, float yprev, T draw, auto out_tag) -> float {
+        constexpr bool OUT = SEG != 1 && decltype(out_tag)::value;
         f2 bcn[NSTATE];
         load_bc(s + 1, bcn);
         float dv, dv_next = 0.f;
@@ -319,10 +323,10 @@
             const f2 e0 = dv2 * a2p[p];
             const f2 a0 = {exp2_hw(e0[0]), exp2_hw(e0[1])};
             hp[p] = a0 * hp[p] + du2 * bcc[p];
-            if constexpr (SEG != 1) yacc = hp[p] * bcc[NSTATE / 2 + p] + yacc;
+            if constexpr (OUT) yacc = hp[p] * bcc[NSTATE / 2 + p] + yacc;
         }
         float yv = 0.f;
-        if constexpr (SEG != 1) {
+        if constexpr (OUT) {
             yv = yacc[0] + yacc[1];
             if constexpr (HASZ) yv *= silu(zv);
             if constexpr (ACC == 1) {
@@ -341,6 +345,17 @@
 
     float pfb0 = 0.f, pfb1 = 0.f;
     const int b_end = SEG ? min(nblk, b_begin + seg_blocks) : nblk;
+    const bool want_mirror = (strand >= want_half) != REV;
+    auto next_want = [&](int after) -> int {
+        int m = 0x7fffffff;
+#pragma unroll
+        for (int q = 0; q < 16; ++q) {
+            const int v = want_mirror ? L - 1 - want.p[q] : want.p[q];
+            if (q < want.n && v > after && v < m) m = v;
+        }
+        return m;
+    };
+    int want_next = SPARSE ? next_want(s_first - 1) : 0;
     for (int b = b_begin; b < b_end; ++b) {
         const int tb0 = REV ? (L - (b + 1) * TB) : b * TB;
 #ifndef PCAD_SCAN_NOPF
@@ -383,8 +398,14 @@
         if constexpr (FUSED) dv_cur = dvs[REV ? TB : 1][lane];
         auto dv_base = [&](int s0) -> const float* { return &dvs[REV ? TB - CH - (s0 - s_begin) : (s0 - s_begin)][lane]; };
         auto run_step = [&](int s, int i, const float* dvp, uint32_t oy, int vy, T uraw, T zraw, T yraw, T draw, uint32_t oys) {
+            if constexpr (SPARSE) {
+                if (s != want_next) { step(s, i, dvp, Elem<T>::to_f32(uraw), 0.f, 0.f, draw, std::false_type{}); return; }
+                want_next = next_want(s);
+                if constexpr (HASZ) zraw = zb_ ? BufIO<T>::load(z_r, vy, oy) : BufIO<T>::load(z_r, voff, (uint32_t)tclamp(s) * rowZ);
+                if constexpr (ACC != 0) yraw = BufIO<T>::load(y_r, vy, oy);
+            }
             const float yv0 = step(s, i, dvp, Elem<T>::to_f32(uraw), HASZ ? Elem<T>::to_f32(zraw) : 0.f,
-                                   ACC != 0 ? Elem<T>::to_f32(yraw) : 0.f, draw);
+                                   ACC != 0 ? Elem<T>::to_f32(yraw) : 0.f, draw, std::true_type{});
             if constexpr (SPLITY && SEG != 1) {
                 float yq = yv0;
                 asm volatile("" : "+v"(yq));
@@ -444,7 +465,7 @@
     }
 }
 
-template <typename T, bool REV, int ACC, bool HASZ, bool FUSED, int PRE, bool BLK8, int SEG = 0, bool ZB = false, bool SPLITY = false>
+template <typename T, bool REV, int ACC, bool HASZ, bool FUSED, int PRE, bool BLK8, int SEG = 0, bool ZB = false, bool SPLITY = false, bool SPARSE = false>
 __global__ __launch_bounds__(64, PRE == 96 ? PCAD_SCAN_OCC96 : PCAD_SCAN_OCC) void scan_kernel(const T* __restrict__ u, const T* __restrict__ z, int64_t ldz,
                                                   const T* __restrict__ dsrc, int64_t ldd,
                                                   const T* __restrict__ Wdt, int Rp,
@@ -452,10 +473,11 @@
                                                   const float* __restrict__ A2, float a_scale,
                                                   const float* __restrict__ Dskip, const float* __restrict__ dbias,
                                                   const T* yin, T* y, int L, int E, int uyb, int zblk, int G, int seg_blocks,
-                                                  float* __restrict__ seg_state, int Lw, bf16_t* __restrict__ ysplit, int dts) {
+                                                  float* __restrict__ seg_state, int Lw, bf16_t* __restrict__ ysplit, int dts,
+                                                  Positions want, int want_half) {
     __shared__ float dvs[TB + 2][64];
-    scan_body<T, REV, ACC, HASZ, FUSED, PRE, BLK8, SEG, ZB, SPLITY>(dvs, (int)blockIdx.x, (int)gridDim.x, u, z, ldz, dsrc, ldd, Wdt, Rp, bc, A2, a_scale,
-                                                                    Dskip, dbias, yin, y, L, E, uyb, zblk, G, seg_blocks, seg_state, Lw, ysplit, dts);
+    scan_body<T, REV, ACC, HASZ, FUSED, PRE, BLK8, SEG, ZB, SPLITY, SPARSE>(dvs, (int)blockIdx.x, (int)gridDim.x, u, z, ldz, dsrc, ldd, Wdt, Rp, bc, A2, a_scale,
+                                                                            Dskip, dbias, yin, y, L, E, uyb, zblk, G, seg_blocks, seg_state, Lw, ysplit, dts, want, want_half);
 }
 
 template <typename T, int ACC, bool HASZ, int PRE, int PHASE, bool SPLITY>
@@ -498,7 +520,8 @@
 
 struct ScanForm {
     bool rev; int acc; bool has_z; int seg; bool splity;
-    bool operator==(const ScanForm& o) const { return rev == o.rev && acc == o.acc && has_z == o.has_z && seg == o.seg && splity == o.splity; }
+    bool sparse = false;
+    bool operator==(const ScanForm& o) const { return rev == o.rev && acc == o.acc && has_z == o.has_z && seg == o.seg && splity == o.splity && sparse == o.sparse; }
 };
 template <typename Row, size_t N, typename Form>
 static auto find_kernel(const Row (&rows)[N], const Form& form) -> decltype(rows[0].kernel) {
@@ -511,13 +534,13 @@
 struct ScanFamily {
     using Kernel = decltype(&scan_kernel<T, false, 0, false, FUSED, PRE, BLK8>);
     struct Row { ScanForm form; Kernel kernel; };
-    template <bool REV, int ACC, bool HZ, int SEG = 0, bool SPLITY = false>
-    static Row row() { return {{REV, ACC, HZ, SEG, SPLITY}, scan_kernel<T, REV, ACC, HZ, FUSED, PRE, BLK8, SEG, ZB && HZ, SPLITY>}; }
-
-    static int slot(const ScanForm& f) { return (((f.seg * 2 + f.rev) * 3 + f.acc) * 2 + f.has_z) * 2 + f.splity; }
+    template <bool REV, int ACC, bool HZ, int SEG = 0, bool SPLITY = false, bool SPARSE = false>
+    static Row row() { return {{REV, ACC, HZ, SEG, SPLITY, SPARSE}, scan_kernel<T, REV, ACC, HZ, FUSED, PRE, BLK8, SEG, ZB && HZ, SPLITY, SPARSE>}; }
+
+    static int slot(const ScanForm& f) { return ((((f.seg * 2 + f.rev) * 3 + f.acc) * 2 + f.has_z) * 2 + f.splity) * 2 + f.sparse; }
     static Kernel kernel(const ScanForm& f) {
-        static const std::array<Kernel, 72> table = [] {
-            std::array<Kernel, 72> t{};
+        static const std::array<Kernel, 144> table = [] {
+            std::array<Kernel, 144> t{};
             auto add = [&t](std::initializer_list<Row> rows) { for (const Row& r : rows) t[slot(r.form)] = r.kernel; };
             add({row<false, 0, false>(), row<false, 0, true>(), row<false, 1, false>(), row<false, 1, true>(), row<false, 2, true>(),
                  row<true, 0, false>(),  row<true, 0, true>(),  row<true, 1, false>(),  row<true, 1, true>(),  row<true, 2, true>()});
@@ -526,6 +549,9 @@
                      row<false, 0, false, 2>(), row<false, 0, true, 2>(), row<true, 0, true, 2>(), row<true, 1, true, 2>(), row<true, 2, true, 2>()});
             if constexpr (std::is_same<T, float>::value && FUSED && BLK8 && ZB)
                 add({row<true, 1, true, 0, true>(), row<true, 2, true, 0, true>()});
+            if constexpr (FUSED && BLK8 && ZB)
+                add({row<false, 0, false, 0, false, true>(), row<false, 0, true, 0, false, true>(),
+                     row<true, 1, true, 0, false, true>(), row<true, 2, true, 0, false, true>()});
             return t;
         }();
         return f.seg >= 0 && f.seg <= 2 && f.acc >= 0 && f.acc <= 2 ? table[slot(f)] : nullptr;
@@ -559,6 +585,9 @@
     const int Sp = a.policy_S > 0 ? a.policy_S : a.S;
     const bool hz = a.z != nullptr, reverse = a.reverse;
     const int accumulate = a.accumulate;
+    if (a.out_rows.n < 0 || a.out_rows.n > 16 || (a.out_rows.n > 0 && (a.ysplit || a.S % 2))) return hipErrorInvalidValue;
+    for (int q = 0; q < a.out_rows.n; ++q)
+        if (a.out_rows.p[q] < 0 || a.out_rows.p[q] >= a.L) return hipErrorInvalidValue;
     if (a.ysplit != nullptr) {
         const bool seg = a.seg_ws && scan_segments(Sp, a.L, a.E, nullptr) > 1;
         if (p.family != ScanFamilyId::F32_ENGINE || !reverse || !hz || (accumulate != 1 && accumulate != 2) || seg || (a.walk_len > 0 && a.walk_len < a.L))
@@ -570,6 +599,7 @@
         int sb = 0;
         const int G = a.seg_ws ? scan_segments(Sp, a.L, a.E, &sb) : 1;
         const bool combo = (!reverse && accumulate == 0) || (reverse && hz && (accumulate == 0 || accumulate == 1 || accumulate == 2));
+        if (G > 1 && a.out_rows.n > 0) return hipErrorInvalidValue;
         if (G > 1 && combo) {
             p.form = {reverse, accumulate, hz, 2, false};
             p.G = G;
@@ -579,6 +609,10 @@
     }
     if (accumulate == 2 && !hz) return hipErrorInvalidValue;
     p.form = {reverse, accumulate == 2 ? 2 : (accumulate ? 1 : 0), hz, 0, false};
+    if (a.out_rows.n > 0) {
+        if (p.family != ScanFamilyId::BF16_ENGINE64 && p.family != ScanFamilyId::BF16_ENGINE96 && p.family != ScanFamilyId::F32_ENGINE) return hipErrorInvalidValue;
+        p.form.sparse = true;
+    }
     return hipSuccess;
 }
 
@@ -594,7 +628,7 @@
         const typename Family::Kernel k = Family::kernel(f);
         if (!k) return hipErrorInvalidValue;
         hipLaunchKernelGGL(k, dim3((unsigned)((int64_t)(E / 64) * S * G)), dim3(64), 0, s, (const T*)d.u, z, a.ldz, dsrc, ldd, Wdt, Rp, d.bc, d.A2, a.a_scale,
-                           d.Dskip, d.dbias, (const T*)a.y, (T*)a.y, L, E, (int)a.uy_blocked, (int)a.z_blocked, G, seg_blocks, seg_ws, walk, ysplit, dts);
+                           d.Dskip, d.dbias, (const T*)a.y, (T*)a.y, L, E, (int)a.uy_blocked, (int)a.z_blocked, G, seg_blocks, seg_ws, walk, ysplit, dts, a.out_rows, S / 2);
         return hipSuccess;
     };
     if (p.G > 1) {
```

Result: no change. 1216 sequences/s, median of 6 (+0.5%).
